# pierrebarbera/epa-ng

Hardware: AMD Instinct MI355X
Metric: query placements/sec (whole node), 512-tip GTR+G4 DNA ref, preplace+thorough (higher is better)
Workload: dtype f64; 1 GPU; cfg2: 512-tip DNA GTR+G4 ref, W=1500, 150 bp reads, dyn-heur 0.99999, preplace+thorough; branches=1021, parallelism=query-shard x1 (weak)

## Files before the change

### epa_ng_amd/api.py

```python
import ctypes as C
import os

import numpy as np

HERE = os.path.dirname(os.path.abspath(__file__))
DEV_SO = os.environ.get("EPA_DEV_SO", os.path.join(HERE, "libepa_dev.so"))

__all__ = ["EpaError", "dev_lib", "device_count", "encode_queries", "Evaluator", "PAIR_DTYPE",
           "RESULT_DTYPE", "ROW_DTYPE", "DEV_SO", "Packed4", "pack_codes_4bit", "unpack_codes_4bit", "Comm",
           "comm_unique_id", "mapped_rccl_path", "comm_set_library", "comm_library_path", "comm_set_default_timeout",
           "pci_id_str", "FLAG_LOOKUP_BLOCKS", "FLAG_LOOKUP_AUTO", "LOOKUP_RESIDENT", "LOOKUP_BLOCKS", "ERR_NO_MEMORY",
           "footprint", "lookup_plan", "set_mem_cap", "quadrature_legendre01", "quadrature_laguerre", "posterior_rule",
           "profile_from_phred"]

FLAG_LOOKUP_BLOCKS = 0x40
FLAG_LOOKUP_AUTO = 0x80
LOOKUP_RESIDENT = 0
LOOKUP_BLOCKS = 1
ERR_NO_MEMORY = -10

PAIR_DTYPE = np.dtype([("branch_id", np.uint32), ("seq_id", np.uint32)])
RESULT_DTYPE = np.dtype([("lnl", np.float64), ("pendant_length", np.float64),
                         ("distal_length", np.float64)])

ROW_DTYPE = np.dtype([("branch_id", np.uint32), ("seq_id", np.uint32), ("lnl", np.float64),
                      ("pendant_length", np.float64), ("distal_length", np.float64)])


class EpaError(RuntimeError):
    def __init__(self, code, msg):
        super().__init__("epa_dev error %d: %s" % (code, msg))
        self.code = code


class _RefDesc(C.Structure):
    _fields_ = [("states", C.c_uint32), ("rate_cats", C.c_uint32), ("sites", C.c_uint32),
                ("branches", C.c_uint32),
                ("eigenvals", C.c_void_p), ("eigenvecs_u", C.c_void_p),
                ("eigenvecs_uinv", C.c_void_p), ("freqs", C.c_void_p), ("rates", C.c_void_p),
                ("rate_weights", C.c_void_p), ("prop_invar", C.c_double),
                ("prox_clv", C.c_void_p), ("prox_scaler", C.c_void_p), ("dist_clv", C.c_void_p),
                ("dist_tipchars", C.c_void_p), ("dist_scaler", C.c_void_p),
                ("branch_length", C.c_void_p),
                ("tipmap", C.c_void_p), ("tipmap_size", C.c_uint32),
                ("blo_min_branch", C.c_double), ("blo_max_branch", C.c_double),
                ("blo_default_branch", C.c_double), ("blo_epsilon", C.c_double),
                ("pendant_default", C.c_double), ("blo_max_rounds", C.c_uint32),
                ("blo_max_newton", C.c_uint32), ("flags", C.c_uint32), ("aa_x_as_n", C.c_uint32),
                ("invariant_state", C.c_void_p)]


class _Stats(C.Structure):
    _fields_ = [("pairs", C.c_uint64), ("rounds", C.c_uint64), ("newton_evals", C.c_uint64),
                ("reverts", C.c_uint64)]


class _Footprint(C.Structure):
    _fields_ = [(n, C.c_uint64) for n in ("reft", "scsum", "lookup", "lookup2", "refi", "misc", "create_temp",
                                          "reference", "bank", "steady", "peak")]


_LIB = None


def dev_lib():
    global _LIB
    if _LIB is None:
        if not os.path.exists(DEV_SO):
            raise ImportError("libepa_dev.so is missing: run `python __graft_entry__.py` "
                              "(build()) -- the HIP extension is the only compute path")
        try:
            import torch
            if torch.cuda.is_available():
                torch.cuda.init()
        except ImportError:
            pass
        L = C.CDLL(DEV_SO)
        L.epa_dev_device_count.restype = C.c_int
        L.epa_dev_create.argtypes = [C.POINTER(_RefDesc), C.c_int, C.POINTER(C.c_void_p)]
        L.epa_dev_destroy.argtypes = [C.c_void_p]
        L.epa_dev_last_error.restype = C.c_char_p
        L.epa_dev_last_error.argtypes = [C.c_void_p]
        L.epa_dev_set_stream.argtypes = [C.c_void_p, C.c_void_p]
        L.epa_dev_build_lookup.argtypes = [C.c_void_p]
        L.epa_dev_set_option.argtypes = [C.c_void_p, C.c_char_p, C.c_int]
        L.epa_encode_queries.argtypes = [C.c_uint32, C.c_uint32, C.c_uint32,
                                         C.POINTER(C.c_char_p), C.c_int, C.c_int, C.c_void_p,
                                         C.c_void_p, C.c_void_p, C.POINTER(C.c_uint32)]
        L.epa_encode_queries_compact.argtypes = [C.c_uint32, C.c_uint32, C.c_uint32,
                                                 C.POINTER(C.c_char_p), C.c_int, C.c_int, C.c_uint32,
                                                 C.c_void_p, C.c_void_p, C.c_void_p,
                                                 C.POINTER(C.c_uint32)]
        L.epa_dev_set_query_layout.argtypes = [C.c_void_p, C.c_uint32]
        L.epa_dev_preplace.argtypes = [C.c_void_p, C.c_void_p, C.c_void_p, C.c_void_p, C.c_uint32,
                                       C.c_void_p]
        L.epa_dev_preplace_bounded.argtypes = [C.c_void_p, C.c_void_p, C.c_void_p, C.c_void_p, C.c_uint32, C.c_uint32,
                                               C.c_void_p, C.c_void_p]
        L.epa_dev_thorough.argtypes = [C.c_void_p, C.c_void_p, C.c_uint64, C.c_void_p, C.c_void_p,
                                       C.c_void_p, C.c_uint32, C.c_void_p, C.POINTER(_Stats)]
        L.epa_dev_score_at.argtypes = [C.c_void_p, C.c_void_p, C.c_void_p, C.c_void_p, C.c_void_p, C.c_uint64,
                                       C.c_void_p, C.c_void_p, C.c_void_p, C.c_uint32, C.c_void_p]
        L.epa_dev_site_lnl.argtypes = [C.c_void_p, C.c_void_p, C.c_void_p, C.c_void_p, C.c_void_p, C.c_uint64,
                                       C.c_void_p, C.c_void_p, C.c_void_p, C.c_uint32, C.c_uint32, C.c_void_p]
        L.epa_dev_rell_support.argtypes = [C.c_void_p, C.c_void_p, C.c_void_p, C.c_void_p, C.c_void_p, C.c_uint64,
                                           C.c_void_p, C.c_void_p, C.c_void_p, C.c_uint32, C.c_void_p, C.c_uint32,
                                           C.c_uint64, C.c_void_p]
        L.epa_dev_rell_tests.argtypes = L.epa_dev_rell_support.argtypes + [C.c_void_p, C.c_void_p]
        L.epa_dev_rell_au.argtypes = L.epa_dev_rell_support.argtypes[:-1] + [C.c_void_p, C.c_uint32, C.c_void_p, C.c_void_p,
                                                                             C.c_void_p]
        L.epa_dev_rell_kh.argtypes = L.epa_dev_rell_tests.argtypes
        L.epa_dev_marginal_like.argtypes = [C.c_void_p, C.c_void_p, C.c_uint64, C.c_void_p, C.c_void_p, C.c_uint32,
                                            C.c_void_p, C.c_void_p, C.c_uint32, C.c_void_p, C.c_void_p, C.c_void_p,
                                            C.c_uint32, C.c_void_p, C.c_void_p]
        L.epa_dev_preplace_profile.argtypes = [C.c_void_p, C.c_void_p, C.c_uint32, C.c_void_p, C.c_void_p, C.c_uint32,
                                               C.c_void_p]
        L.epa_dev_thorough_profile.argtypes = [C.c_void_p, C.c_void_p, C.c_uint64, C.c_void_p, C.c_uint32, C.c_void_p,
                                               C.c_void_p, C.c_uint32, C.c_void_p, C.POINTER(_Stats)]
        L.epa_dev_score_at_profile.argtypes = [C.c_void_p, C.c_void_p, C.c_void_p, C.c_void_p, C.c_void_p, C.c_uint64,
                                               C.c_void_p, C.c_uint32, C.c_void_p, C.c_void_p, C.c_uint32, C.c_void_p]
        L.epa_dev_site_lnl_profile.argtypes = [C.c_void_p, C.c_void_p, C.c_void_p, C.c_void_p, C.c_void_p, C.c_uint64,
                                               C.c_void_p, C.c_uint32, C.c_void_p, C.c_void_p, C.c_uint32, C.c_uint32,
                                               C.c_void_p]
        L.epa_dev_place_chunk_profile.argtypes = [C.c_void_p, C.c_void_p, C.c_uint32, C.c_void_p, C.c_void_p, C.c_uint32,
                                                  C.c_double, C.c_void_p, C.c_void_p, C.c_uint64, C.POINTER(C.c_uint64),
                                                  C.POINTER(_Stats)]
        L.epa_profile_from_phred.argtypes = [C.c_uint32, C.c_uint32, C.c_uint32, C.c_void_p, C.c_void_p, C.c_void_p,
                                             C.c_void_p]
        L.epa_quadrature_legendre01.argtypes = [C.c_uint32, C.c_void_p, C.c_void_p]
        L.epa_quadrature_laguerre.argtypes = [C.c_uint32, C.c_void_p, C.c_void_p]
        L.epa_dev_set_heuristic.argtypes = [C.c_void_p, C.c_int, C.c_double]
        L.epa_dev_set_query_packing.argtypes = [C.c_void_p, C.c_int]
        L.epa_pack_codes_4bit.argtypes = [C.c_void_p, C.c_uint32, C.c_uint32, C.c_void_p]
        L.epa_unpack_codes_4bit.argtypes = [C.c_void_p, C.c_uint32, C.c_uint32, C.c_void_p]
        L.epa_dev_select_candidates.argtypes = [C.c_void_p, C.c_void_p, C.c_uint32, C.c_double,
                                                C.c_void_p, C.c_uint64, C.POINTER(C.c_uint64)]
        L.epa_dev_place_chunk.argtypes = [C.c_void_p, C.c_void_p, C.c_void_p, C.c_void_p, C.c_uint32,
                                          C.c_uint32, C.c_double, C.c_void_p, C.c_void_p,
                                          C.c_uint64, C.POINTER(C.c_uint64), C.POINTER(_Stats)]
        L.epa_dev_dedup_queries.argtypes = [C.c_void_p, C.c_void_p, C.c_void_p, C.c_void_p, C.c_uint32, C.c_void_p,
                                            C.c_void_p, C.POINTER(C.c_uint32)]
        L.epa_dev_place_chunk_dedup.argtypes = [C.c_void_p, C.c_void_p, C.c_void_p, C.c_void_p, C.c_uint32, C.c_uint32,
                                                C.c_double, C.c_void_p, C.c_void_p, C.c_uint64, C.POINTER(C.c_uint64),
                                                C.POINTER(_Stats), C.c_void_p, C.c_void_p, C.POINTER(C.c_uint32)]
        L.epa_dev_chunk_stage.argtypes = [C.c_void_p, C.c_int, C.c_void_p, C.c_void_p, C.c_void_p, C.c_uint32]
        L.epa_dev_chunk_launch.argtypes = [C.c_void_p, C.c_int, C.c_uint32, C.c_double, C.c_void_p,
                                           C.c_void_p, C.c_uint64, C.c_uint32]
        L.epa_dev_chunk_launch_begin.argtypes = [C.c_void_p, C.c_int, C.c_uint32, C.c_double, C.c_void_p,
                                           C.c_void_p, C.c_uint64, C.c_uint32]
        L.epa_dev_chunk_launch_end.argtypes = [C.c_void_p, C.c_int]
        L.epa_dev_chunk_launch_many_begin.argtypes = [C.c_void_p, C.POINTER(C.c_int), C.c_int, C.c_uint32, C.c_double,
                                                      C.c_uint64, C.c_uint32]
        L.epa_dev_chunk_launch_many.argtypes = L.epa_dev_chunk_launch_many_begin.argtypes
        L.epa_dev_chunk_finish.argtypes = [C.c_void_p, C.c_int, C.POINTER(C.c_void_p),
                                           C.POINTER(C.c_void_p), C.POINTER(C.c_uint64), C.POINTER(_Stats)]
        L.epa_dev_tree_logl.argtypes = [C.c_void_p, C.c_uint32, C.POINTER(C.c_double)]
        L.epa_dev_place_all.argtypes = [C.c_void_p, C.c_void_p, C.c_void_p, C.c_void_p, C.c_uint32,
                                        C.c_uint32, C.c_double, C.c_int, C.c_uint32, C.c_uint32,
                                        C.c_void_p, C.c_void_p, C.c_void_p, C.c_void_p,
                                        C.POINTER(_Stats)]
        L.epa_comm_get_unique_id.argtypes = [C.c_void_p]
        L.epa_comm_create.argtypes = [C.c_void_p, C.c_void_p, C.c_int, C.c_int, C.c_uint32, C.c_int,
                                      C.POINTER(C.c_void_p)]
        L.epa_comm_destroy.argtypes = [C.c_void_p]
        L.epa_comm_destroy.restype = None
        L.epa_dev_gather_results.argtypes = [C.c_void_p, C.c_void_p, C.c_void_p, C.c_void_p, C.c_uint64,
                                             C.c_uint32, C.POINTER(C.c_uint64)]
        L.epa_dev_gather_slot.argtypes = [C.c_void_p, C.c_void_p, C.c_int, C.c_uint32, C.POINTER(C.c_uint64)]
        L.epa_comm_collect.argtypes = [C.c_void_p, C.c_uint64, C.POINTER(C.c_void_p), C.POINTER(C.c_uint32),
                                       C.POINTER(C.c_uint64)]
        L.epa_comm_flush.argtypes = [C.c_void_p, C.c_void_p, C.POINTER(C.c_uint64), C.POINTER(C.c_uint32)]
        L.epa_comm_carried_rows.argtypes = [C.c_void_p]
        L.epa_comm_carried_rows.restype = C.c_uint64
        L.epa_dev_gather_rows.argtypes = [C.c_void_p, C.c_void_p, C.c_void_p, C.c_uint64, C.POINTER(C.c_uint64)]
        L.epa_dev_place_all_rows.argtypes = [C.c_void_p, C.c_void_p, C.c_void_p, C.c_void_p, C.c_uint32, C.c_uint32, C.c_double,
                                             C.c_int, C.c_uint32, C.c_uint32, C.c_uint32, C.POINTER(C.c_void_p),
                                             C.POINTER(C.c_uint64), C.c_void_p]
        L.epa_comm_abort.argtypes = [C.c_void_p]
        L.epa_comm_abort.restype = None
        L.epa_comm_set_library.argtypes = [C.c_char_p]
        L.epa_comm_library_path.restype = C.c_char_p
# ... 189 lines not shown
                    held.append(a)
                    arr[i] = a.ctypes.data
            return arr, held

        pc, h1 = ptr_array(prox_clv, np.float64)
        dc, h2 = ptr_array(dist_clv, np.float64)
        ps, h3 = ptr_array(prox_scaler, np.uint32)
        ds, h4 = ptr_array(dist_scaler, np.uint32)
        dt, h5 = ptr_array(dist_tip, np.uint8)
        tm = np.ascontiguousarray(tipmap, dtype=np.uint32) if tipmap is not None else None
        d = _RefDesc()
        d.states, d.rate_cats, d.sites, d.branches = states, self.c, W, B
        d.eigenvals, d.eigenvecs_u, d.eigenvecs_uinv = (keep[0].ctypes.data, keep[1].ctypes.data,
                                                       keep[2].ctypes.data)
        d.freqs, d.rates, d.rate_weights = keep[3].ctypes.data, keep[4].ctypes.data, keep[5].ctypes.data
        d.prop_invar = float(pinv)
        inv = None
        if invariant_state is not None:
            inv = np.ascontiguousarray(invariant_state, dtype=np.int8)
            d.invariant_state = inv.ctypes.data
        d.prox_clv = C.cast(pc, C.c_void_p)
        d.prox_scaler = C.cast(ps, C.c_void_p)
        d.dist_clv = C.cast(dc, C.c_void_p)
        d.dist_tipchars = C.cast(dt, C.c_void_p) if dist_tip is not None else None
        d.dist_scaler = C.cast(ds, C.c_void_p)
        d.branch_length = keep[6].ctypes.data
        if tm is not None:
            d.tipmap, d.tipmap_size = tm.ctypes.data, len(tm)
        d.aa_x_as_n = int(aa_x_as_n)
        d.flags = int(flags)
        h = C.c_void_p()
        rc = L.epa_dev_create(C.byref(d), device, C.byref(h))
        if rc:
            raise EpaError(rc, L.epa_dev_last_error(None).decode())
        self.h = h
        self.L = L
        self.last_stats = None

    def close(self):
        if getattr(self, "h", None):
            self.L.epa_dev_destroy(self.h)
            self.h = None

    def __del__(self):
        self.close()

    def _check(self, rc):
        if rc:
            raise EpaError(rc, self.L.epa_dev_last_error(self.h).decode())

    def set_stream(self, stream_ptr):
        self._check(self.L.epa_dev_set_stream(self.h, stream_ptr))

    def set_option(self, key, value=1):
        self._check(self.L.epa_dev_set_option(self.h, key.encode(), int(value)))

    def build_lookup(self):
        self._check(self.L.epa_dev_build_lookup(self.h))

    def _layout(self, codes):
        packed = isinstance(codes, Packed4)
        row = codes.stride if packed else (int(codes.shape[1]) if len(codes.shape) == 2 else self.W)
        self._check(self.L.epa_dev_set_query_layout(self.h, 0 if row == self.W else row))
        self._check(self.L.epa_dev_set_query_packing(self.h, 4 if packed else 8))

    def preplace(self, codes, win_begin, win_span, Q=None, out=None):
        Q = len(win_begin) if Q is None else Q
        if out is None:
            out = np.empty((Q, self.B), np.float64)
        self._layout(codes)
        self._check(self.L.epa_dev_preplace(self.h, _ptr(codes), _ptr(win_begin), _ptr(win_span),
                                            Q, _ptr(out)))
        return out

    def preplace_bounded(self, codes, win_begin, win_span, max_span, seg_keys=False):
        Q = len(win_begin)
        out = np.empty((Q, self.B), np.float64)
        keys = np.zeros((Q, ((self.B + 63) // 64 + 7) // 8 * 8), np.uint64) if seg_keys else None
        self._layout(codes)
        self._check(self.L.epa_dev_preplace_bounded(self.h, _ptr(codes), _ptr(win_begin), _ptr(win_span), Q,
                                                    int(max_span), _ptr(out), _ptr(keys)))
        return (out, keys) if seg_keys else out

    def thorough(self, pairs, codes, win_begin, win_span, Q=None, n_pairs=None, out=None):
        Q = len(win_begin) if Q is None else Q
        n = len(pairs) if n_pairs is None else n_pairs
        if out is None:
            out = np.empty(n, RESULT_DTYPE)
        st = _Stats()
        self._layout(codes)
        self._check(self.L.epa_dev_thorough(self.h, _ptr(pairs), n, _ptr(codes), _ptr(win_begin),
                                            _ptr(win_span), Q, _ptr(out), C.byref(st)))
        self.last_stats = {"pairs": st.pairs, "rounds": st.rounds,
                           "newton_evals": st.newton_evals, "reverts": st.reverts}
        return out

    def _entries(self, pairs, pendant, distal, proximal, codes, win_begin, Q, stream_id=None):
        n, Q = len(pairs), (len(win_begin) if Q is None else Q)
        host = (np.ndarray, list, tuple)
        pendant, distal, proximal = (np.ascontiguousarray(a, dtype=np.float64) if isinstance(a, host) else a
                                     for a in (pendant, distal, proximal))
        if isinstance(stream_id, host):
            stream_id = np.ascontiguousarray(stream_id, dtype=np.uint64)
        self._layout(codes)
        return n, Q, pendant, distal, proximal, stream_id

    @staticmethod
    def _want(who, want, table):
        want = tuple(want)
        unknown = [w for w in want if w not in table]
        if unknown:
            raise ValueError("%s: unknown output %r" % (who, unknown[0]))
        return {w: np.empty(*table[w]) for w in want}

    def score_at(self, pairs, pendant, distal, codes, win_begin, win_span, proximal=None, Q=None, out=None):
        n, Q, pendant, distal, proximal, _ = self._entries(pairs, pendant, distal, proximal, codes, win_begin, Q)
        if out is None:
            out = np.empty(n, np.float64)
        self._check(self.L.epa_dev_score_at(self.h, _ptr(pairs), _ptr(pendant), _ptr(distal), _ptr(proximal), n,
                                            _ptr(codes), _ptr(win_begin), _ptr(win_span), Q, _ptr(out)))
        return out

    def site_lnl(self, pairs, pendant, distal, codes, win_begin, win_span, proximal=None, pitch=None, Q=None, out=None):
        n, Q, pendant, distal, proximal, _ = self._entries(pairs, pendant, distal, proximal, codes, win_begin, Q)
        if pitch is None:
            pitch = int(np.max(np.asarray(win_span)[:Q])) if Q else 0
        if out is None:
            out = np.empty((n, int(pitch)), np.float64)
        self._check(self.L.epa_dev_site_lnl(self.h, _ptr(pairs), _ptr(pendant), _ptr(distal), _ptr(proximal), n,
                                            _ptr(codes), _ptr(win_begin), _ptr(win_span), Q, int(pitch), _ptr(out)))
        return out

    def marginal_like(self, pairs, codes, win_begin, win_span, x_frac, x_logw, p_len, p_logw, Q=None, out=None, grid=False):
        n, Q = self._entries(pairs, None, None, None, codes, win_begin, Q)[:2]
        x_frac, x_logw, p_len, p_logw = (np.ascontiguousarray(a, dtype=np.float64) for a in (x_frac, x_logw, p_len, p_logw))
        if x_frac.shape != x_logw.shape or p_len.shape != p_logw.shape or x_frac.ndim != 1 or p_len.ndim != 1:
            raise ValueError("marginal_like: nodes and log weights must be 1-d arrays of equal length")
        Kx, Kp = len(x_frac), len(p_len)
        if out is None:
            out = np.empty(n, np.float64)
        g = np.empty((n, Kx, Kp), np.float64) if grid else None
        self._check(self.L.epa_dev_marginal_like(self.h, _ptr(pairs), n, _ptr(x_frac), _ptr(x_logw), Kx, _ptr(p_len),
                                                 _ptr(p_logw), Kp, _ptr(codes), _ptr(win_begin), _ptr(win_span), Q,
                                                 _ptr(out), _ptr(g)))
        return (out, g) if grid else out

    def rell_support(self, pairs, pendant, distal, codes, win_begin, win_span, replicates, seed=1, stream_id=None,
                     proximal=None, Q=None, out=None):
        n, Q, pendant, distal, proximal, stream_id = self._entries(pairs, pendant, distal, proximal, codes, win_begin, Q,
                                                                   stream_id)
        if out is None:
            out = np.empty(n, np.float64)
        self._check(self.L.epa_dev_rell_support(self.h, _ptr(pairs), _ptr(pendant), _ptr(distal), _ptr(proximal), n,
                                                _ptr(codes), _ptr(win_begin), _ptr(win_span), Q, _ptr(stream_id),
                                                int(replicates), int(seed), _ptr(out)))
        return out

    def rell_tests(self, pairs, pendant, distal, codes, win_begin, win_span, replicates, seed=1, stream_id=None,
                   proximal=None, want=("support", "elw", "p_sh"), Q=None):
        out = self._want("rell_tests", want, {w: ((len(pairs),), np.float64) for w in ("support", "elw", "p_sh")})
        n, Q, pendant, distal, proximal, stream_id = self._entries(pairs, pendant, distal, proximal, codes, win_begin, Q,
                                                                   stream_id)
        self._check(self.L.epa_dev_rell_tests(self.h, _ptr(pairs), _ptr(pendant), _ptr(distal), _ptr(proximal), n,
                                              _ptr(codes), _ptr(win_begin), _ptr(win_span), Q, _ptr(stream_id),
                                              int(replicates), int(seed), _ptr(out.get("support")), _ptr(out.get("elw")),
                                              _ptr(out.get("p_sh"))))
# ... 405 lines not shown
```

### epa_ng_amd/csrc/chunk.hip

```cpp
#include "epa_dev_internal.hpp"

#include <string.h>

#include <algorithm>

static int chunk_body_begin(epa_ctx* ctx, const uint8_t* d_codes, const uint32_t* d_begin, const uint32_t* d_span,
                            uint32_t Q, uint32_t max_span, double threshold, epa_pair* d_pairs,
                            uint64_t max_pairs, uint32_t* rb, SelectPending* sp, epa_result* d_res = nullptr,
                            unsigned long long* d_stats = nullptr) {
  const uint32_t pitch = (ctx->B + 7u) & ~7u;
  PreTable t{(double*)epa_scratch(ctx, SLOT_TABLE, sizeof(double) * (size_t)Q * pitch), pitch};
  if (!t.lnl) return epa_fail(ctx, EPA_ERR_HIP, "hipMalloc(chunk table)");
  const uint32_t nseg = (ctx->B + 63) / 64;
  if (nseg <= 64 && ctx->heur_mode == 0) {
    t.segp = (nseg + 7u) & ~7u;
    t.segmax = (unsigned long long*)epa_scratch(ctx, SLOT_SEGMAX, sizeof(unsigned long long) * (size_t)Q * t.segp);
    if (!t.segmax) return epa_fail(ctx, EPA_ERR_HIP, "hipMalloc(segment maxima)");
  }
  const uint32_t* pre_status = nullptr;
  int rc = launch_preplace(ctx, d_codes, d_begin, d_span, Q, t, max_span, &pre_status);
  if (!rc) rc = launch_select_begin(ctx, t, pre_status, Q, threshold, d_pairs, max_pairs, d_span, rb, sp);
  const bool behind_rb = !rc && d_stats && sp->d_rb && sp->bitmap && max_pairs <= 0xffffffffull;
  if (behind_rb) {
    rc = launch_select_emit(ctx, sp);
    if (!rc) rc = epa_zero_async(ctx, d_stats, 128, epa_th_ctr(ctx), epa_th_ctr(ctx) ? 64 : 0);
    if (!rc) {
      ctx->clean_stats[ctx->bank] = d_stats;
      ctx->clean_ctr[ctx->bank] = epa_th_ctr(ctx) != nullptr;
    }
  }
  if (behind_rb && !rc && d_res) {
    const bool off = !ctx->opt.queued_thorough;
    const int cls = epa_span_class(ctx->s, max_span);
    const bool eligible = !off && ctx->s == 4 && !ctx->generic_thorough && ctx->dna.ng == 1 && epa_th_ctr(ctx) &&
                          epa_tip_class_ok(cls);
    if (eligible) {
      rc = launch_select_emit(ctx, sp);
      if (!rc && ctx->clean_stats[ctx->bank] == d_stats) ctx->clean_stats[ctx->bank] = nullptr;
      else if (!rc) rc = epa_zero_async(ctx, d_stats, 128);
      if (!rc) {
        const int q = launch_thorough_queued(ctx, d_pairs, sp->d_rb, max_pairs, d_codes, d_begin, d_span, max_span, d_res, d_stats);
        if (q == -2) return EPA_ERR_HIP;
        sp->queued_cls = q;
      }
    }
  }
  return rc;
}

static int chunk_body_end(epa_ctx* ctx, SelectPending* sp, const uint8_t* d_codes, const uint32_t* d_begin,
                          const uint32_t* d_span, uint32_t max_span, epa_pair* d_pairs, epa_result* d_res,
                          unsigned long long* d_stats, uint64_t* n_out) {
  uint64_t n = 0;
  int rc = launch_select_end(ctx, sp, &n);
  if (rc) return rc;
  rc = select_check_status(ctx, sp);
  if (rc) return rc;
  *n_out = n;
  if (sp->queued_cls >= 0 && sp->rb[RB_HIST + sp->queued_cls] + sp->rb[RB_HIST + epa_tip_class(sp->queued_cls)] == (uint32_t)n) return EPA_OK;
  if (ctx->clean_stats[ctx->bank] == d_stats && sp->queued_cls < 0) ctx->clean_stats[ctx->bank] = nullptr;
  else {
    ctx->clean_stats[ctx->bank] = nullptr;
    rc = epa_zero_async(ctx, d_stats, 128);
    if (rc) return rc;
  }
  if (n == 0) return EPA_OK;
  const bool hist_ok = sp->have_hist && (sp->tip_split || !epa_tipd_active(ctx));
  return launch_thorough(ctx, d_pairs, n, d_codes, d_begin, d_span, max_span, d_res, d_stats,
                         hist_ok ? sp->cls_hist : nullptr);
}

static int chunk_body(epa_ctx* ctx, const uint8_t* d_codes, const uint32_t* d_begin, const uint32_t* d_span,
                      uint32_t Q, uint32_t max_span, double threshold, epa_pair* d_pairs, epa_result* d_res,
                      uint64_t max_pairs, unsigned long long* d_stats, uint64_t* n_out) {
  uint32_t rb[64] = {};
  SelectPending sp;
  int rc = chunk_body_begin(ctx, d_codes, d_begin, d_span, Q, max_span, threshold, d_pairs, max_pairs, rb, &sp, d_res, d_stats);
  if (rc) return rc;
  return chunk_body_end(ctx, &sp, d_codes, d_begin, d_span, max_span, d_pairs, d_res, d_stats, n_out);
}

int chunk_stats(epa_ctx* ctx, uint64_t n, const unsigned long long* hst, epa_thorough_stats* stats) {
  epa_xcd_feedback(ctx, n, hst);
  ctx->last_stats.pairs = n;
  ctx->last_stats.rounds = hst[0];
  ctx->last_stats.newton_evals = hst[1];
  ctx->last_stats.reverts = hst[2];
  if (stats) *stats = ctx->last_stats;
  if (hst[3])
    return epa_fail(ctx, EPA_ERR_NEG_INF,
                    "-INF logl at branch " + std::to_string((uint32_t)(hst[4] >> 32)) +
                        " with sequence " + std::to_string((uint32_t)(hst[4] & 0xffffffffu)));
  return EPA_OK;
}

extern "C" int epa_dev_place_chunk(epa_ctx* ctx, const uint8_t* q_codes, const uint32_t* win_begin,
                                   const uint32_t* win_span, uint32_t Q, uint32_t max_span,
                                   double threshold, epa_pair* pairs, epa_result* results,
                                   uint64_t max_pairs, uint64_t* n_pairs, epa_thorough_stats* stats) {
  if (!ctx || !q_codes || !win_begin || !win_span || !pairs || !results || !n_pairs)
    return epa_fail(ctx, EPA_ERR_INVALID_ARG, "null argument");
// ... 460 lines not shown
```

### epa_ng_amd/csrc/epa_dev.hip

```cpp
#include "epa_dev_internal.hpp"

#include <math.h>
#include <string.h>

#include <algorithm>
#include <numeric>
#include <atomic>
#include <thread>

static thread_local std::string g_create_err;

int epa_fail(epa_ctx* ctx, int code, const std::string& msg) {
  if (ctx) ctx->err = msg; else g_create_err = msg;
  return code;
}

namespace {
__global__ void __launch_bounds__(256) k_zero(uint4* __restrict__ a, size_t na, uint4* __restrict__ b, size_t nb) {
  const size_t stride = (size_t)gridDim.x * 256, i0 = (size_t)blockIdx.x * 256 + threadIdx.x;
  const uint4 z = make_uint4(0u, 0u, 0u, 0u);
  for (size_t i = i0; i < na; i += stride) a[i] = z;
  for (size_t i = i0; i < nb; i += stride) b[i] = z;
}
}
// ... 481 lines not shown
}

extern "C" int epa_quadrature_legendre01(uint32_t K, double* nodes, double* log_weights) {
  if (K < 1 || K > 64 || !nodes || !log_weights) return EPA_ERR_INVALID_ARG;
  std::vector<double> d(K, 0.0), o(K > 1 ? K - 1 : 0), x;
  for (uint32_t i = 1; i < K; ++i) o[i - 1] = (double)i / std::sqrt(4.0 * i * i - 1.0);
  tridiag_eigenvalues(d, o, x);
  for (uint32_t j = 0; j < K; ++j) {
    double t = x[j], dp = 1.0;
    for (int it = 0; it < 3; ++it) {
      double p0 = 1.0, p1 = t;
      for (uint32_t n = 1; n < K; ++n) { const double p2 = ((2.0 * n + 1.0) * t * p1 - n * p0) / (n + 1.0); p0 = p1; p1 = p2; }
      dp = K * (t * p1 - p0) / (t * t - 1.0);
      if (it < 2) t -= p1 / dp;
    }
    nodes[j] = 0.5 * (1.0 + t);
    log_weights[j] = -std::log((1.0 - t) * (1.0 + t)) - 2.0 * std::log(std::fabs(dp));
  }
  const double norm = log_sum_exp(log_weights, K);
  for (uint32_t j = 0; j < K; ++j) log_weights[j] -= norm;
  return EPA_OK;
}

extern "C" int epa_quadrature_laguerre(uint32_t K, double* nodes, double* log_weights) {
  if (K < 1 || K > 64 || !nodes || !log_weights) return EPA_ERR_INVALID_ARG;
  std::vector<double> d(K), o(K > 1 ? K - 1 : 0), x;
  for (uint32_t i = 0; i < K; ++i) d[i] = 2.0 * i + 1.0;
  for (uint32_t i = 1; i < K; ++i) o[i - 1] = (double)i;
  tridiag_eigenvalues(d, o, x);
  for (uint32_t j = 0; j < K; ++j) {
    double t = x[j], lm = 1.0;
    for (int it = 0; it < 3; ++it) {
      double l0 = 1.0, l1 = 1.0 - t;
      for (uint32_t n = 1; n < K; ++n) { const double l2 = ((2.0 * n + 1.0 - t) * l1 - n * l0) / (n + 1.0); l0 = l1; l1 = l2; }
      lm = l0;
      if (it < 2) t -= l1 * t / (K * (l1 - l0));
    }
    nodes[j] = t;
    log_weights[j] = std::log(t) - 2.0 * std::log((double)K) - 2.0 * std::log(std::fabs(lm));
  }
  const double norm = log_sum_exp(log_weights, K);
  for (uint32_t j = 0; j < K; ++j) log_weights[j] -= norm;
  return EPA_OK;
}

extern "C" int epa_dev_device_count(void) {
  int n = 0;
  if (hipGetDeviceCount(&n) != hipSuccess) { (void)hipGetLastError(); return 0; }
  return n;
}

extern "C" const char* epa_dev_last_error(const epa_ctx* ctx) {
  return ctx ? ctx->err.c_str() : g_create_err.c_str();
}

extern "C" int epa_dev_set_query_layout(epa_ctx* ctx, uint32_t code_stride) {
  if (!ctx) return EPA_ERR_INVALID_ARG;
  ctx->code_stride = code_stride;
  return EPA_OK;
}

extern "C" int epa_dev_set_option(epa_ctx* ctx, const char* key, int value) {
  if (!ctx || !key) return EPA_ERR_INVALID_ARG;
  if (strcmp(key, "lookup_block") == 0) {
    if (!ctx->lookup_blocks) return epa_fail(ctx, EPA_ERR_INVALID_ARG, "set_option: lookup_block needs a context in the blocked lookup layout");
    if (value <= 0 || (value & 63)) return epa_fail(ctx, EPA_ERR_INVALID_ARG, "set_option: lookup_block must be a positive multiple of 64");
    for (void* p : ctx->blk_buf)
      if (p) return epa_fail(ctx, EPA_ERR_INVALID_ARG, "set_option: lookup_block must be set before the first preplacement");
    ctx->lookup_block = (uint32_t)value;
    return EPA_OK;
  }
  const bool dedup_key = strcmp(key, "dedup_key_bits") == 0;
  if (dedup_key || strcmp(key, "dedup_sort_bits") == 0) {
    if (value < 0 || value > 64) return epa_fail(ctx, EPA_ERR_INVALID_ARG, std::string("set_option: ") + key + " must be 0 .. 64");
    (dedup_key ? ctx->opt.dedup_key_bits : ctx->opt.dedup_sort_bits) = value;
    return EPA_OK;
  }
  struct Entry { const char* name; int EpaOptions::*field; };
  static const Entry table[] = {
      {"thorough_generic", &EpaOptions::thorough_generic}, {"preplace_generic", &EpaOptions::preplace_generic},
      {"select_full_rows", &EpaOptions::select_full_rows}, {"select_sort", &EpaOptions::select_sort},
      {"queued_thorough", &EpaOptions::queued_thorough},   {"xcd_balance", &EpaOptions::xcd_balance},
      {"aa_valu", &EpaOptions::aa_valu},                   {"timers", &EpaOptions::timers},
      {"newton_lds", &EpaOptions::newton_lds},             {"tip_distal", &EpaOptions::tip_distal}};
  for (const Entry& e : table)
    if (strcmp(key, e.name) == 0) {
      ctx->opt.*e.field = value;
      ctx->generic_thorough = ctx->generic_native || ctx->opt.thorough_generic != 0;
      return EPA_OK;
    }
  return epa_fail(ctx, EPA_ERR_INVALID_ARG, std::string("set_option: unknown key '") + key + "'");
}

extern "C" int epa_dev_set_heuristic(epa_ctx* ctx, int mode, double param) {
  if (!ctx) return EPA_ERR_INVALID_ARG;
  if (mode < EPA_HEUR_DYNAMIC || mode > EPA_HEUR_BASEBALL)
    return epa_fail(ctx, EPA_ERR_INVALID_ARG, "set_heuristic: unknown mode");
  if (mode == EPA_HEUR_FIXED && !(param >= 0.0 && param <= 1.0))
    return epa_fail(ctx, EPA_ERR_INVALID_ARG, "set_heuristic: the fraction must lie in [0, 1]");
  ctx->heur_mode = mode;
  ctx->heur_param = param;
  return EPA_OK;
}

extern "C" int epa_dev_set_query_packing(epa_ctx* ctx, int bits) {
  if (!ctx) return EPA_ERR_INVALID_ARG;
  if (bits != 8 && bits != 4) return epa_fail(ctx, EPA_ERR_INVALID_ARG, "set_query_packing: 8 or 4 bits per code");
  if (bits == 4 && ctx->s != 4)
    return epa_fail(ctx, EPA_ERR_UNSUPPORTED, "set_query_packing: the 4-bit format holds nucleotide codes only");
  ctx->code_packed4 = bits == 4;
  return EPA_OK;
}

extern "C" int epa_pack_codes_4bit(const uint8_t* codes, uint32_t Q, uint32_t stride, uint8_t* packed) {
  if (!codes || !packed) return EPA_ERR_INVALID_ARG;
  const size_t ps = ((size_t)stride + 1) / 2;
  const unsigned cap = g_encode_threads.load(std::memory_order_relaxed);
  const unsigned hw = cap ? cap : std::max(1u, std::thread::hardware_concurrency());
  const unsigned nt = (unsigned)std::min<uint64_t>(std::min(hw, 32u), std::max<uint64_t>(1, (uint64_t)Q * stride >> 20));
  std::vector<int> bad(nt, 0);
  auto work = [&](unsigned t) {
    const uint32_t q0 = (uint32_t)((uint64_t)Q * t / nt), q1 = (uint32_t)((uint64_t)Q * (t + 1) / nt);
    unsigned over = 0;
    for (uint32_t q = q0; q < q1; ++q) {
      const uint8_t* r = codes + (size_t)q * stride;
      uint8_t* o = packed + (size_t)q * ps;
      for (uint32_t p = 0; p < stride / 2; ++p) {
        const uint8_t hi = r[2 * p], lo = r[2 * p + 1];
        over |= hi | lo;
        o[p] = (uint8_t)((hi << 4) | lo);
      }
      if (stride & 1) { const uint8_t hi = r[stride - 1]; over |= hi; o[ps - 1] = (uint8_t)(hi << 4); }
    }
    bad[t] = over > 15;
  };
  if (nt == 1) work(0);
  else {
    std::vector<std::thread> th;
    for (unsigned t = 0; t < nt; ++t) th.emplace_back(work, t);
    for (auto& x : th) x.join();
  }
  for (unsigned t = 0; t < nt; ++t) if (bad[t]) return EPA_ERR_INVALID_ARG;
  return EPA_OK;
}

extern "C" int epa_unpack_codes_4bit(const uint8_t* packed, uint32_t Q, uint32_t stride, uint8_t* codes) {
  if (!codes || !packed) return EPA_ERR_INVALID_ARG;
  const size_t ps = ((size_t)stride + 1) / 2;
  for (uint32_t q = 0; q < Q; ++q)
    for (uint32_t i = 0; i < stride; ++i) {
      const uint8_t b = packed[(size_t)q * ps + i / 2];
      codes[(size_t)q * stride + i] = (i & 1) ? (b & 15u) : (b >> 4);
    }
  return EPA_OK;
}

extern "C" int epa_dev_set_stream(epa_ctx* ctx, void* s) {
  if (!ctx) return EPA_ERR_INVALID_ARG;
  ctx->stream = (hipStream_t)s;
  return EPA_OK;
}

extern "C" void epa_dev_destroy(epa_ctx* ctx) {
  if (!ctx) return;
  (void)hipSetDevice(ctx->device);
  (void)hipDeviceSynchronize();
  for (int i = 0; i < epa_ctx::N_BANKS * epa_ctx::N_SCRATCH; ++i) if (ctx->scratch[i]) (void)hipFree(ctx->scratch[i]);
  if (ctx->refT) (void)hipFree(ctx->refT);
  if (ctx->scSum) (void)hipFree(ctx->scSum);
  if (ctx->blen) (void)hipFree(ctx->blen);
  if (ctx->lookup) (void)hipFree(ctx->lookup);
  if (ctx->lookup2) (void)hipFree(ctx->lookup2);
  if (ctx->prof_tab) (void)hipFree(ctx->prof_tab);
  for (void* p : ctx->blk_buf) if (p) (void)hipFree(p);
  for (auto& v : ctx->blk_ev) for (hipEvent_t e : v) if (e) (void)hipEventDestroy(e);
  if (ctx->th_ctr) (void)hipFree(ctx->th_ctr);
  for (hipEvent_t e : ctx->ev_rb) if (e) (void)hipEventDestroy(e);
  if (ctx->refI) (void)hipFree(ctx->refI);
  if (ctx->cinv) (void)hipFree(ctx->cinv);
  if (ctx->resc0) (void)hipFree(ctx->resc0);
  if (ctx->tip_row) (void)hipFree(ctx->tip_row);
  if (ctx->tipmask) (void)hipFree(ctx->tipmask);
  if (ctx->tipd) (void)hipFree(ctx->tipd);
  for (hipStream_t st : ctx->side_stream) if (st) (void)hipStreamDestroy(st);
  for (hipEvent_t e : ctx->ev_fork) if (e) (void)hipEventDestroy(e);
  for (hipEvent_t e : ctx->ev_join) if (e) (void)hipEventDestroy(e);
  if (ctx->dmodel) (void)hipFree(ctx->dmodel);
  for (ChunkSlot& sl : ctx->slots) {
    if (sl.h_in) (void)hipHostFree(sl.h_in);
    if (sl.h_out) (void)hipHostFree(sl.h_out);
    if (sl.h_stats) (void)hipHostFree(sl.h_stats);
    if (sl.h_sel) (void)hipHostFree(sl.h_sel);
    if (sl.d_in) (void)hipFree(sl.d_in);
    if (sl.d_unpacked) (void)hipFree(sl.d_unpacked);
    if (sl.d_pairs) (void)hipFree(sl.d_pairs);
    if (sl.d_res) (void)hipFree(sl.d_res);
    if (sl.d_stats) (void)hipFree(sl.d_stats);
    if (sl.d_merge) (void)hipFree(sl.d_merge);
    if (sl.d_gpairs) (void)hipFree(sl.d_gpairs);
    if (sl.d_gres) (void)hipFree(sl.d_gres);
    if (sl.d_goff) (void)hipFree(sl.d_goff);
    if (sl.h_goff) (void)hipHostFree(sl.h_goff);
    for (hipEvent_t e : {sl.ev_up, sl.ev_done, sl.ev_down, sl.ev_base}) if (e) (void)hipEventDestroy(e);
    if (sl.stream) (void)hipStreamDestroy(sl.stream);
  }
  if (ctx->copy_stream) (void)hipStreamDestroy(ctx->copy_stream);
  if (ctx->down_stream) (void)hipStreamDestroy(ctx->down_stream);
  std::vector<EvTimer*> ts = {&ctx->t_lookup};
  for (auto& bk : ctx->t_bank) for (auto& t : bk) ts.push_back(&t);
  for (auto* t : ts) { if (t->a) (void)hipEventDestroy(t->a); if (t->b) (void)hipEventDestroy(t->b); }
  delete ctx;
}

static int precompute_from_tree(epa_ctx* ctx, const epa_tree_desc* t, const uint32_t* d_tipmap);

static int padded_cats(int s, int c_in, uint32_t flags, bool from_tree) {
  int c = (c_in == 1 || c_in == 2) ? 4 : c_in;
  if (s == 4 && c_in >= 3 && (c_in & 3)) c = (c_in + 3) & ~3;
  if (s == 20 && (c_in == 3 || (c_in >= 5 && c_in <= 7))) c = (c_in + 3) & ~3;
  if (c_in >= 3 && c != c_in && (flags & EPA_FLAG_RATE_SCALERS) && !from_tree) c = c_in;
  return c;
}

static bool tuned_thorough_shape(int s, int c, uint32_t flags, bool zero0) {
  const bool sliding = !(flags & EPA_FLAG_RAXML_BLO);
  const bool dna_groups = s == 4 && (c & 3) == 0 && c <= 16;
  const bool tuned_local = (s == 4 && zero0) || s == 20;
  const bool tuned_cats = c == 4 || (dna_groups && sliding && zero0) || (s == 20 && c == 8);
  return tuned_cats && (sliding || tuned_local) &&
         !(flags & (EPA_FLAG_NEWTON_SLOW_BISECT | EPA_FLAG_NEWTON_STRICT_DF | EPA_FLAG_KEEP_EIGENVALUES));
}

static std::atomic<uint64_t> g_mem_cap{0};
extern "C" void epa_dev_set_mem_cap(uint64_t bytes) { g_mem_cap.store(bytes, std::memory_order_relaxed); }

constexpr uint32_t EPA_BLOCK_DEFAULT = 1024;
constexpr int EPA_PLAN_BANKS = 4;

extern "C" int epa_dev_footprint(uint32_t states, uint32_t rate_cats, uint64_t sites, uint64_t branches, int flags,
                                 int from_tree, uint32_t block_branches, int banks, epa_footprint* out) {
  if (!out || !(states == 4 || states == 20) || rate_cats < 1 || rate_cats > EPA_MAX_CATS || !sites || !branches ||
      sites > 0xffffffffull || branches > 0xffffffffull || banks < 0 || (block_branches & 63u))
    return epa_fail(nullptr, EPA_ERR_INVALID_ARG, "footprint: bad shape");
  const uint64_t s = states, W = sites, B = branches;
  const uint64_t c = (uint64_t)padded_cats((int)states, (int)rate_cats, (uint32_t)flags, from_tree != 0);
  const bool blocks = (flags & EPA_FLAG_LOOKUP_BLOCKS) != 0;
  const bool tuned = tuned_thorough_shape((int)s, (int)c, (uint32_t)flags, !(flags & EPA_FLAG_KEEP_EIGENVALUES));
  epa_footprint f;
  memset(&f, 0, sizeof(f));
  f.reft = 8 * 2 * B * c * s * W;
  f.scsum = 4 * B * W;
  if (!blocks) {
    f.lookup = 8 * B * W * (s == 4 ? 16 : 24);
    f.lookup2 = s == 4 ? 8 * B * 2 * ((W + 1) / 2) * 36 : 0;
    f.refi = tuned ? 8 * B * c * s * W + B * W : 0;
// ... 679 lines not shown
}

extern "C" int epa_dev_build_lookup(epa_ctx* ctx) {
  if (!ctx) return EPA_ERR_INVALID_ARG;
  if (ctx->lookup_built || ctx->lookup_blocks) return EPA_OK;
  EPA_HIP(ctx, hipSetDevice(ctx->device));
  int rc = launch_build_lookup(ctx);
  if (rc) return rc;
  EPA_HIP(ctx, hipStreamSynchronize(ctx->stream));
  ctx->lookup_built = true;
  return EPA_OK;
}

const uint32_t* host_view(const uint32_t* p, size_t n, std::vector<uint32_t>& buf, hipStream_t st) {
  if (!epa_is_device_ptr(p)) return p;
  buf.resize(n);
  (void)hipStreamSynchronize(st);
  if (hipMemcpy(buf.data(), p, n * sizeof(uint32_t), hipMemcpyDeviceToHost) != hipSuccess)
    return nullptr;
  return buf.data();
}

static int check_windows(epa_ctx* ctx, const uint32_t* hb, const uint32_t* hs, uint32_t Q,
                         uint32_t* max_span, bool allow_empty = false) {
  uint32_t mx = 0;
  for (uint32_t q = 0; q < Q; ++q) {
    if (hs[q] == 0 && !allow_empty)
      return epa_fail(ctx, EPA_ERR_QUERY_ALL_GAP,
                      "Sequence " + std::to_string(q) + " does not appear to have any non-gap sites!");
    if ((uint64_t)hb[q] + hs[q] > ctx->W)
      return epa_fail(ctx, EPA_ERR_QUERY_WIDTH,
                      "Query sequence length not same as reference alignment!");
    mx = std::max(mx, hs[q]);
  }
  if (ctx->code_stride && mx > ctx->code_stride)
    return epa_fail(ctx, EPA_ERR_INVALID_ARG, "a window is longer than the compact code stride");
  *max_span = mx;
  return EPA_OK;
}

extern "C" int epa_dev_preplace(epa_ctx* ctx, const uint8_t* q_codes, const uint32_t* win_begin,
                                const uint32_t* win_span, uint32_t Q, double* lnl) {
  return epa_dev_preplace_bounded(ctx, q_codes, win_begin, win_span, Q, 0, lnl, nullptr);
}

extern "C" int epa_dev_preplace_bounded(epa_ctx* ctx, const uint8_t* q_codes, const uint32_t* win_begin,
                                        const uint32_t* win_span, uint32_t Q, uint32_t max_span, double* lnl,
                                        uint64_t* seg_keys) {
  if (!ctx || !q_codes || !win_begin || !win_span || !lnl)
    return epa_fail(ctx, EPA_ERR_INVALID_ARG, "null argument");
  if (Q == 0) return EPA_OK;
  EPA_HIP(ctx, hipSetDevice(ctx->device));
  int rc = epa_dev_build_lookup(ctx);
  if (rc) return rc;
  if (max_span > ctx->W) max_span = ctx->W;
  if (max_span && !epa_is_device_ptr(win_span))
    for (uint32_t q = 0; q < Q; ++q)
      if (win_span[q] > max_span) return epa_fail(ctx, EPA_ERR_INVALID_ARG, "preplace: a window is longer than max_span");
  const uint32_t nseg = (ctx->B + 63) / 64, segp = (nseg + 7u) & ~7u;
  unsigned long long* d_seg = nullptr;
  if (seg_keys) {
    if (nseg > 64) return epa_fail(ctx, EPA_ERR_INVALID_ARG, "preplace: segment maxima exist up to 4096 branches");
    d_seg = (unsigned long long*)epa_scratch(ctx, SLOT_SEGMAX, sizeof(unsigned long long) * (size_t)Q * segp);
    if (!d_seg) return epa_fail(ctx, EPA_ERR_HIP, "hipMalloc(segment maxima)");
  }
  const uint8_t* d_codes = epa_codes_to_device(ctx, q_codes, Q);
  const uint32_t* d_begin = (const uint32_t*)epa_to_device(ctx, SLOT_BEGIN, win_begin, sizeof(uint32_t) * Q);
  const uint32_t* d_span = (const uint32_t*)epa_to_device(ctx, SLOT_SPAN, win_span, sizeof(uint32_t) * Q);
  if (!d_codes || !d_begin || !d_span) return epa_fail(ctx, EPA_ERR_HIP, "query upload failed");
  const bool out_dev = epa_is_device_ptr(lnl);
  double* d_lnl = out_dev ? lnl : (double*)epa_scratch(ctx, SLOT_TABLE, sizeof(double) * (size_t)Q * ctx->B);
  if (!d_lnl) return epa_fail(ctx, EPA_ERR_HIP, "hipMalloc(lnl)");
  const uint32_t* d_status = nullptr;
  rc = launch_preplace(ctx, d_codes, d_begin, d_span, Q, PreTable{d_lnl, ctx->B, d_seg, segp}, max_span, &d_status);
  if (rc) return rc;
  if (!out_dev)
    EPA_HIP(ctx, hipMemcpyAsync(lnl, d_lnl, sizeof(double) * (size_t)Q * ctx->B,
                                hipMemcpyDeviceToHost, ctx->stream));
  if (d_seg)
    EPA_HIP(ctx, hipMemcpyAsync(seg_keys, d_seg, sizeof(unsigned long long) * (size_t)Q * segp,
                                epa_is_device_ptr(seg_keys) ? hipMemcpyDeviceToDevice : hipMemcpyDeviceToHost, ctx->stream));
  EPA_HIP(ctx, hipStreamSynchronize(ctx->stream));
  return preplace_check_status(ctx, d_status);
}

extern "C" int epa_dev_thorough(epa_ctx* ctx, const epa_pair* pairs, uint64_t n_pairs,
                                const uint8_t* q_codes, const uint32_t* win_begin,
                                const uint32_t* win_span, uint32_t Q, epa_result* out,
                                epa_thorough_stats* stats) {
  if (!ctx || !q_codes || !win_begin || !win_span || (n_pairs && (!pairs || !out)))
    return epa_fail(ctx, EPA_ERR_INVALID_ARG, "null argument");
  if (stats) memset(stats, 0, sizeof(*stats));
  if (n_pairs == 0) return EPA_OK;
  EPA_HIP(ctx, hipSetDevice(ctx->device));
  if (ctx->refI) {
    int brc = epa_dev_build_lookup(ctx);
    if (brc) return brc;
  }
  std::vector<uint32_t> hb_buf, hs_buf;
  const uint32_t* hb = host_view(win_begin, Q, hb_buf, ctx->stream);
  const uint32_t* hs = host_view(win_span, Q, hs_buf, ctx->stream);
  if (!hb || !hs) return epa_fail(ctx, EPA_ERR_HIP, "cannot read window arrays");
  uint32_t max_span = 0;
  int rc = check_windows(ctx, hb, hs, Q, &max_span);
  if (rc) return rc;
  if (!epa_is_device_ptr(pairs)) {
    for (uint64_t i = 0; i < n_pairs; ++i)
      if (pairs[i].branch_id >= ctx->B || pairs[i].seq_id >= Q)
        return epa_fail(ctx, EPA_ERR_INVALID_ARG, "pair index out of range");
  }
  const uint8_t* d_codes = epa_codes_to_device(ctx, q_codes, Q);
  const uint32_t* d_begin = (const uint32_t*)epa_to_device(ctx, SLOT_BEGIN, win_begin, sizeof(uint32_t) * Q);
  const uint32_t* d_span = (const uint32_t*)epa_to_device(ctx, SLOT_SPAN, win_span, sizeof(uint32_t) * Q);
  const epa_pair* d_pairs = (const epa_pair*)epa_to_device(ctx, SLOT_PAIRS, pairs, sizeof(epa_pair) * n_pairs);
  if (!d_codes || !d_begin || !d_span || !d_pairs)
    return epa_fail(ctx, EPA_ERR_HIP, "thorough input upload failed");
  const bool out_dev = epa_is_device_ptr(out);
  epa_result* d_out = out_dev ? out : (epa_result*)epa_scratch(ctx, SLOT_RESULTS, sizeof(epa_result) * n_pairs);
  unsigned long long* d_stats = (unsigned long long*)epa_scratch(ctx, SLOT_STATS, 256);
  if (!d_out || !d_stats) return epa_fail(ctx, EPA_ERR_HIP, "hipMalloc(thorough out)");
  rc = epa_zero_async(ctx, d_stats, 128);
  if (rc) return rc;
  rc = launch_thorough(ctx, d_pairs, n_pairs, d_codes, d_begin, d_span, max_span, d_out, d_stats);
  if (rc) return rc;
  unsigned long long hst[16];
  if (!out_dev)
    EPA_HIP(ctx, hipMemcpyAsync(out, d_out, sizeof(epa_result) * n_pairs, hipMemcpyDeviceToHost,
                                ctx->stream));
  if (!out_dev || stats) {
    EPA_HIP(ctx, hipMemcpyAsync(hst, d_stats, 128, hipMemcpyDeviceToHost, ctx->stream));
    EPA_HIP(ctx, hipStreamSynchronize(ctx->stream));
    return chunk_stats(ctx, n_pairs, hst, stats);
  }
  return EPA_OK;
}


namespace {

struct EntryArgs {
  const epa_pair* pairs;
  const double *pendant, *distal, *proximal;
  uint64_t n;
  const uint8_t* q_codes;
  const uint32_t *win_begin, *win_span;
  uint32_t Q;
  const double* prof = nullptr;
  uint32_t prof_stride = 0;
};

struct EntryCall {
  epa_ctx* ctx;
  const char* who;
  EntryArgs a;
  EntryStage st;
  std::vector<uint32_t> hb_buf, hs_buf;
  const uint64_t* d_sid = nullptr;
  bool empty = false;
  struct Out { void *user, *dev; size_t bytes; } out[3] = {};
  int n_out = 0;

  int stage() {
    const uint32_t* hb = host_view(a.win_begin, a.Q, hb_buf, ctx->stream);
    st.h_span = host_view(a.win_span, a.Q, hs_buf, ctx->stream);
    if (!hb || !st.h_span) return epa_fail(ctx, EPA_ERR_HIP, "cannot read window arrays");
    int rc = a.prof ? (int)EPA_OK : check_windows(ctx, hb, st.h_span, a.Q, &st.max_span, true);
// ... 558 lines not shown
```

### epa_ng_amd/csrc/epa_dev_internal.hpp

```cpp
#pragma once

#include <hip/hip_runtime.h>
#include <stdint.h>

#include <string>
#include <vector>

#include <rocprim/device/device_radix_sort.hpp>

#include "epa_dev.h"

using epa_radix_cfg = rocprim::radix_sort_config<rocprim::default_config, rocprim::default_config,
                                                 rocprim::default_config, 0>;

#define EPA_MAX_STATES 20
#define EPA_MAX_CATS 16
#define EPA_MAX_COLS 24
#define EPA_GRID_Y 65535u

struct ModelDNA {
  double U[16];
  double Ui[16];
  double lam[4];
  double rate[16];
  double w[16];
  double pi[4];
  int ng;
};

struct BloConsts {
  double min_branch, max_branch, default_branch, epsilon, pendant_default;
  uint32_t max_rounds, max_newton;
  uint32_t sliding;
  uint32_t newton_variant;
};

struct ModelDev {
  int s, c, ncols;
  double U[EPA_MAX_STATES * EPA_MAX_STATES];
  double Ui[EPA_MAX_STATES * EPA_MAX_STATES];
  double lam[EPA_MAX_STATES];
  double pi[EPA_MAX_STATES];
  double rate[EPA_MAX_CATS];
  double w[EPA_MAX_CATS];
  uint32_t colmask[EPA_MAX_COLS];
  double qt[EPA_MAX_COLS * EPA_MAX_STATES];
};

struct EvTimer {
  hipEvent_t a = nullptr, b = nullptr;
  bool valid = false;
};

constexpr int EPA_N_CLS = 12;
constexpr int EPA_N_CLSX = 17;

enum EpaReadback : int {
  RB_TOTAL = 0,
  RB_STATUS = RB_TOTAL + 1,
  RB_HIST = RB_STATUS + 8,
  RB_TIP_SPLIT = 30,
  RB_WINDOW = 32,
  RB_WORDS = RB_WINDOW + 4,
};
enum EpaSelStatus : int {
  SEL_OVERFLOW = 2,
  SEL_HIST = 8,
  SEL_TIP_TOTAL = 40,
  SEL_READBACK = 64,
  SEL_WORDS = 128,
};
static_assert(RB_TOTAL == 0 && RB_STATUS == 1 && RB_HIST == 9 && RB_TIP_SPLIT == 30 && RB_WINDOW == 32 && RB_WORDS == 36,
              "the read-back block's layout is shared with queued kernels: move a word everywhere or nowhere");
static_assert(RB_HIST + EPA_N_CLSX <= RB_TIP_SPLIT && RB_TIP_SPLIT < RB_WINDOW, "read-back fields overlap");
static_assert(SEL_HIST == 8 && SEL_TIP_TOTAL == 40 && SEL_READBACK == 64, "the selection's status block moved");
static_assert(RB_HIST - RB_STATUS == SEL_HIST, "k_pack_readback copies status words and histogram in one run");
static_assert(SEL_HIST + EPA_N_CLS <= SEL_TIP_TOTAL && SEL_TIP_TOTAL < SEL_READBACK && SEL_READBACK + RB_WORDS <= SEL_WORDS,
              "status block fields overlap");

struct PreTable {
  double* lnl = nullptr;
  uint32_t pitch = 0;
  unsigned long long* segmax = nullptr;
  uint32_t segp = 0;
};

struct SelectPending {
  PreTable table;
  const uint32_t* pre_status = nullptr;
  uint32_t Q = 0, cap = 0;
  double threshold = 0.0;
  epa_pair* d_pairs = nullptr;
  uint64_t max_pairs = 0;
  const uint32_t* d_span = nullptr;
  unsigned long long *stage = nullptr, *keys_a = nullptr, *keys_b = nullptr;
  uint32_t *counts = nullptr, *offsets = nullptr;
  uint32_t *bitmap = nullptr, *boffs = nullptr;
  uint32_t wpr = 0;
  void* temp = nullptr;
  size_t sort_bytes = 0;
  uint32_t* rb = nullptr;
  bool have_status = false;
  hipEvent_t ev_rb = nullptr;
  const uint32_t* d_rb = nullptr;
  bool emitted = false;
  int queued_cls = -1;
  uint32_t cls_hist[EPA_N_CLSX] = {};
  bool have_hist = false;
  bool tip_split = false;
};

enum class SlotState : int {
  Free,
  Staged,
  Begun,
  Launched,
  GroupMember,
};
constexpr int EPA_MAX_GROUP = 8;

struct ChunkInputs {
  const uint8_t* codes;
  const uint32_t *begin, *span;
};

struct __attribute__((visibility("hidden"))) ChunkSlot {
  void* h_in = nullptr;
  size_t h_in_sz = 0;
  void* d_in = nullptr;
  const uint8_t* x_codes = nullptr;
  const uint32_t* x_begin = nullptr;
  const uint32_t* x_span = nullptr;
  size_t d_in_sz = 0;
  uint8_t* d_unpacked = nullptr;
  size_t d_unpacked_sz = 0;
  size_t codes_bytes = 0;
  uint32_t Q = 0, stride = 0;
  bool packed4 = false;
  epa_pair* d_pairs = nullptr;
  epa_result* d_res = nullptr;
  size_t d_pairs_sz = 0, d_res_sz = 0;
  void* h_out = nullptr;
  size_t h_out_sz = 0;
  unsigned long long* h_stats = nullptr;
  unsigned long long* d_stats = nullptr;
  hipEvent_t ev_up = nullptr, ev_done = nullptr, ev_down = nullptr, ev_base = nullptr;
  hipStream_t stream = nullptr;
  const epa_pair* out_pairs = nullptr;
  const epa_result* out_res = nullptr;
  uint64_t n = 0;
  SlotState state = SlotState::Free;
  bool unfinished() const { return state == SlotState::Begun || state == SlotState::Launched || state == SlotState::GroupMember; }
  ChunkInputs staged_inputs() const {
    if (x_codes) return {x_codes, x_begin, x_span};
    const char* d = (const char*)d_in;
    const uint32_t* b = (const uint32_t*)(d + codes_bytes);
    return {(const uint8_t*)d, b, b + Q};
  }
  SelectPending sel;
  uint32_t* h_sel = nullptr;
  const uint8_t* l_codes = nullptr;
  const uint32_t *l_begin = nullptr, *l_span = nullptr;
  epa_pair* l_pairs = nullptr;
  epa_result* l_res = nullptr;
  uint32_t l_max_span = 0, l_flags = 0;
  int leader = -1;
  int g_index = 0;
  int g_n = 0;
  int g_left = 0;
  int g_slots[EPA_MAX_GROUP] = {};
  uint32_t g_qoff[EPA_MAX_GROUP + 1] = {};
  uint32_t own_Q = 0;
  const uint8_t* own_x_codes = nullptr;
  const uint32_t *own_x_begin = nullptr, *own_x_span = nullptr;
  void* d_merge = nullptr;
  size_t d_merge_sz = 0;
  epa_pair* d_gpairs = nullptr;
  epa_result* d_gres = nullptr;
  size_t g_cap = 0;
  uint32_t* d_goff = nullptr;
  uint32_t* h_goff = nullptr;

  void lead_merged(uint32_t total, const uint8_t* codes, const uint32_t* begin, const uint32_t* span) {
    own_Q = Q; own_x_codes = x_codes; own_x_begin = x_begin; own_x_span = x_span;
    Q = total; x_codes = codes; x_begin = begin; x_span = span;
  }
  void restore_own() { Q = own_Q; x_codes = own_x_codes; x_begin = own_x_begin; x_span = own_x_span; }
  void group_begun(ChunkSlot* all, const int* slots, int n, const uint32_t* qoff) {
    g_n = n;
    for (int i = 0; i <= n; ++i) g_qoff[i] = qoff[i];
    for (int i = 0; i < n; ++i) {
      g_slots[i] = slots[i];
      all[slots[i]].leader = slots[0];
      all[slots[i]].g_index = i;
      if (i) all[slots[i]].state = SlotState::GroupMember;
    }
  }
  void group_launched(ChunkSlot* all) {
    restore_own();
    g_left = g_n;
    for (int i = 1; i < g_n; ++i) {
      all[g_slots[i]].state = SlotState::Launched;
      all[g_slots[i]].l_flags = l_flags;
    }
  }
  void launch_over(ChunkSlot* all, SlotState to) {
    state = to;
    if (g_n <= 1) return;
    restore_own();
    for (int i = 0; i < g_n; ++i) {
      all[g_slots[i]].leader = -1;
      if (i) all[g_slots[i]].state = to;
    }
    g_n = 0;
    g_left = 0;
  }
};

struct EpaOptions {
  int thorough_generic = 0;
  int preplace_generic = 0;
  int select_full_rows = 0;
  int select_sort = 0;
  int queued_thorough = 0;
  int xcd_balance = 1;
  int aa_valu = 0;
  int timers = 1;
  int newton_lds = 0;
  int tip_distal = 1;
  int dedup_key_bits = 64;
  int dedup_sort_bits = 32;
};

struct epa_ctx {
  int device = 0;
  EpaOptions opt;
  int n_cu = 256;
  hipStream_t stream = nullptr;
  std::string err;

  int s = 0, c = 0, ncols = 0;
  int c_in = 0;
  uint32_t W = 0, B = 0;
  ModelDev hmodel;
  ModelDev* dmodel = nullptr;
  ModelDNA dna;
  bool dna_zero0 = false;
  bool rate_scalers = false;
  bool generic_thorough = false;
  bool generic_native = false;
  BloConsts blo;
  int aa_x_as_n = 0;
  uint32_t code_stride = 0;

  double* refT = nullptr;
  uint32_t* scSum = nullptr;
  double* blen = nullptr;
  double* lookup = nullptr;
  double* refI = nullptr;
  uint8_t* resc0 = nullptr;
  double* cinv = nullptr;
  double inv_w0 = 0.0;
  double* lookup2 = nullptr;
  uint32_t* tip_row = nullptr;
  uint8_t* tipmask = nullptr;
  double* tipd = nullptr;
  bool lookup_built = false;
  double* prof_tab = nullptr;
  bool lookup_blocks = false;
  uint32_t lookup_block = 1024;
  std::vector<double> h_blen;

  static constexpr int N_SCRATCH = 26;
  static constexpr int N_SLOTS = 24;
  static constexpr int N_BANKS = 1 + N_SLOTS;
  int bank = 0;
  void* scratch[N_BANKS * N_SCRATCH] = {};
  size_t scratch_sz[N_BANKS * N_SCRATCH] = {};

  uint32_t select_cap = 64;
  uint32_t* th_ctr = nullptr;
  bool code_packed4 = false;
  int heur_mode = 0;
  double heur_param = 0.0;

  hipStream_t copy_stream = nullptr, down_stream = nullptr;
  ChunkSlot slots[N_SLOTS];

  enum { T_PREPLACE = 0, T_THOROUGH = 1, T_SELECT = 2, T_SCORE = 3, T_SITES = 4, T_RELL = 5, T_MARGINAL = 6, T_RELL_TESTS = 7, T_RELL_AU = 8, T_RELL_KH = 9, T_PREPLACE_PROFILE = 10, T_DEDUP = 11, N_TIMERS = 12 };
  EvTimer t_lookup;
  std::vector<hipEvent_t> blk_ev[N_BANKS];
  uint32_t blk_ev_n[N_BANKS] = {};
  void* blk_buf[N_BANKS] = {};
  size_t blk_sz[N_BANKS] = {};
  EvTimer t_bank[N_BANKS][N_TIMERS];
  uint32_t xcd_cum[9] = {0u, 1u << 17, 2u << 17, 3u << 17, 4u << 17, 5u << 17, 6u << 17, 7u << 17, 1u << 20};
  double xcd_w[8] = {0.125, 0.125, 0.125, 0.125, 0.125, 0.125, 0.125, 0.125};
  double last_sclk_mhz = 0.0;
  bool xstamp_ok = false;
  hipEvent_t ev_rb[N_BANKS] = {};
  hipStream_t side_stream[N_BANKS] = {};
  hipEvent_t ev_fork[N_BANKS] = {}, ev_join[N_BANKS] = {};
  const void* clean_stats[N_BANKS] = {};
  bool clean_ctr[N_BANKS] = {};
  int t_last[N_TIMERS] = {};
  epa_thorough_stats last_stats{};
};

int epa_fail(epa_ctx* ctx, int code, const std::string& msg);
void* epa_scratch(epa_ctx* ctx, int slot, size_t bytes);
inline size_t align256(size_t x) { return (x + 255) & ~(size_t)255; }
struct Carver {
  char* base = nullptr;
  size_t off = 0;
  void* tail(size_t bytes) { char* p = base ? base + off : nullptr; off += bytes; return p; }
  template <typename T> T* take(size_t n) { return static_cast<T*>(tail(align256(sizeof(T) * n))); }
};
inline uint32_t* epa_th_ctr(epa_ctx* ctx) { return ctx->th_ctr ? ctx->th_ctr + 64 * ctx->bank : nullptr; }
int epa_zero_async(epa_ctx* ctx, void* p, size_t bytes, void* p2 = nullptr, size_t bytes2 = 0);
inline int epa_th_ctr_reset(epa_ctx* ctx, size_t bytes = 64) {
  if (ctx->clean_ctr[ctx->bank]) { ctx->clean_ctr[ctx->bank] = false; return 0; }
  return epa_zero_async(ctx, epa_th_ctr(ctx), bytes);
}
bool epa_is_device_ptr(const void* p);
const void* epa_to_device(epa_ctx* ctx, int slot, const void* p, size_t bytes);
const uint8_t* epa_codes_to_device(epa_ctx* ctx, const uint8_t* q_codes, uint32_t Q);
__attribute__((visibility("hidden"))) void launch_unpack4(hipStream_t st, const uint8_t* d_packed, uint8_t* d_codes, uint32_t Q, uint32_t stride);
__attribute__((visibility("hidden"))) const uint32_t* host_view(const uint32_t* p, size_t n, std::vector<uint32_t>& buf, hipStream_t st);
void epa_xcd_feedback(epa_ctx* ctx, uint64_t n_pairs, const unsigned long long* hst);
__attribute__((visibility("hidden"))) int chunk_stats(epa_ctx* ctx, uint64_t n, const unsigned long long* hst, epa_thorough_stats* stats);
#define EPA_XSTAMP_MASK 0x7ffffffffffull
void epa_timer_start(epa_ctx* ctx, EvTimer& t);
void epa_timer_stop(epa_ctx* ctx, EvTimer& t);
inline EvTimer& epa_t(epa_ctx* ctx, int which) { ctx->t_last[which] = ctx->bank; return ctx->t_bank[ctx->bank][which]; }

#define EPA_HIP(ctx, call)                                                               \
  do {                                                                                    \
    hipError_t e__ = (call);                                                              \
    if (e__ != hipSuccess)                                                                \
      return epa_fail(ctx, EPA_ERR_HIP, std::string(#call) + ": " + hipGetErrorString(e__)); \
  } while (0)

enum EpaSlot : int {
  SLOT_CODES = 0,
  SLOT_BEGIN = 1,
  SLOT_SPAN = 2,
  SLOT_OUT = 3,
  SLOT_PAIRS = 4,
  SLOT_CLV_PROX = 0,
  SLOT_CLV_DIST = 1,
  SLOT_TIPMAP = 2,
  SLOT_SCALER_PROX = 3,
  SLOT_SCALER_DIST = 4,
  SLOT_TABLE = 3,
  SLOT_RESULTS = 5,
  SLOT_PREPLACE = 6,
  SLOT_STATS = 6,
  SLOT_SELECT = 7,
  SLOT_NEWTON = 7,
  SLOT_CLASS_SORT = 8,
  SLOT_TREE_LNL = 9,
  SLOT_TH_TIMING = 9,
  SLOT_SEGMAX = 10,
  SLOT_PACKED4 = 10,
  SLOT_ROWS_OUT = 11,
  SLOT_ROWS = 12,
  SLOT_PENDANT = 7,
  SLOT_DISTAL = 8,
  SLOT_PROXIMAL = 9,
  SLOT_MG_RULE = 7,
  SLOT_MG_WAVES = 9,
  SLOT_RELL_SORT = 13,
  SLOT_RELL_BOUNDS = 14,
  SLOT_RELL_GROUPS = 15,
  SLOT_RELL_ROWS = 16,
  SLOT_RELL_STREAMS = 17,
  SLOT_RELL_TESTS = 18,
  SLOT_RELL_AU = 19,
  SLOT_RELL_KH = 20,
  SLOT_PROFILE = 21,
  SLOT_PROFILE_EIGEN = 22,
  SLOT_DEDUP = 23,
  SLOT_DEDUP_IN = 24,
  SLOT_DEDUP_ROWS = 25,
};

struct EntryStage {
  const epa_pair* d_pairs = nullptr;
  const double *d_pen = nullptr, *d_dis = nullptr, *d_prx = nullptr;
  uint64_t n = 0;
  const uint8_t* d_codes = nullptr;
  const uint32_t *d_begin = nullptr, *d_span = nullptr;
  const uint32_t* h_span = nullptr;
  const double* d_qe = nullptr;
  uint32_t qe_stride = 0;
  uint32_t Q = 0;
  uint32_t max_span = 0;
};

__host__ __device__ inline bool epa_tip_class_ok(int cls) { return cls <= 2 || cls == 10 || cls == 11; }
__host__ __device__ inline int epa_tip_class(int cls) { return cls <= 2 ? 12 + cls : cls == 10 ? 15 : cls == 11 ? 16 : cls; }
__host__ __device__ inline int epa_base_class(int key) { return key < 12 ? key : key <= 14 ? key - 12 : key == 15 ? 10 : 11; }
inline bool epa_tipd_active(const epa_ctx* ctx) {
  return ctx->tip_row && ctx->opt.tip_distal && ctx->s == 4 && !ctx->generic_thorough && ctx->dna.ng == 1 &&
         ctx->dna_zero0 && ctx->blo.sliding && !ctx->cinv;
}
constexpr uint32_t EPA_AA_LDS_MAX_SPAN = 102;
__host__ __device__ inline int epa_span_class(int states, uint32_t span) {
  if (states != 4) return span <= 64 ? 0 : span <= 128 ? 1 : span <= 192 ? 2 : 3;
  if (span > 64 && span <= 96) return 10;
  if (span > 128 && span <= 160) return 11;
  const uint32_t nch = (span + 63) / 64;
  return nch <= 4 ? (nch ? (int)nch - 1 : 0) : nch <= 6 ? 4 : nch <= 8 ? 5 : nch <= 12 ? 6 : nch <= 16 ? 7 : nch <= 24 ? 8 : 9;
}

int launch_transform(epa_ctx* ctx, const double* d_clv_or_null, const uint8_t* d_tip_or_null,
                     const uint32_t* d_tipmap, uint32_t tipmap_size, double* dst);
int launch_build_lookup(epa_ctx* ctx);
int launch_build_lookup2(epa_ctx* ctx);
uint32_t epa_block_branches(const epa_ctx* ctx);
size_t epa_block_bytes(int s, uint32_t W, uint32_t blk, size_t* off2);
void* epa_block_buffer(epa_ctx* ctx);
int launch_build_lookup_block(epa_ctx* ctx, uint32_t b0, uint32_t nb, double* blk_lookup);
int launch_build_lookup2_block(epa_ctx* ctx, uint32_t nb, const double* blk_lookup, double* blk_lookup2);
int launch_preplace(epa_ctx* ctx, const uint8_t* d_codes, const uint32_t* d_begin, const uint32_t* d_span, uint32_t Q,
                    const PreTable& t, uint32_t max_span, const uint32_t** d_status);
int preplace_check_status(epa_ctx* ctx, const uint32_t* d_status);
__attribute__((visibility("hidden"))) int preplace_window_error(epa_ctx* ctx, const uint32_t* st);
__attribute__((visibility("hidden"))) void launch_scan_counts(epa_ctx* ctx, uint32_t* cnt, uint32_t K, const uint32_t* tip_row = nullptr,
                                                               uint32_t* tip_total = nullptr);
int launch_thorough(epa_ctx* ctx, const epa_pair* d_pairs, uint64_t n_pairs, const uint8_t* d_codes,
                    const uint32_t* d_begin, const uint32_t* d_span, uint32_t max_span,
                    epa_result* d_out, unsigned long long* d_stats,
                    const uint32_t* cls_hist = nullptr);
int launch_thorough_queued(epa_ctx* ctx, const epa_pair* d_pairs, const uint32_t* d_spec, uint64_t max_pairs,
                           const uint8_t* d_codes, const uint32_t* d_begin, const uint32_t* d_span, uint32_t max_span,
                           epa_result* d_out, unsigned long long* d_stats);
int launch_select_emit(epa_ctx* ctx, SelectPending* sp);
int launch_thorough_aa(epa_ctx* ctx, const epa_pair* d_pairs, const uint32_t* d_order, uint64_t n_pairs,
                       const uint8_t* d_codes, const uint32_t* d_begin, const uint32_t* d_span,
                       uint32_t max_span, bool want_lds, epa_result* d_out, unsigned long long* d_stats);
int launch_thorough_generic(epa_ctx* ctx, const epa_pair* d_pairs, uint64_t n_pairs, const uint8_t* d_codes,
                            const uint32_t* d_begin, const uint32_t* d_span, uint32_t max_span,
                            epa_result* d_out, unsigned long long* d_stats,
                            const uint32_t* d_order = nullptr, bool caller_times = false,
                            const double* d_qe = nullptr, uint32_t qe_stride = 0);
int launch_thorough_aa_mfma(epa_ctx* ctx, const epa_pair* d_pairs, const uint32_t* d_order, uint64_t n_pairs,
                            const uint8_t* d_codes, const uint32_t* d_begin, const uint32_t* d_span,
                            uint32_t max_span, epa_result* d_out, unsigned long long* d_stats);
__attribute__((visibility("hidden"))) uint32_t epa_column_mask(int s, int col);
__attribute__((visibility("hidden"))) int epa_profile_stage(epa_ctx* ctx, const char* who, const double* prof, uint32_t stride,
                                                            const uint32_t* hb, const uint32_t* hs, const uint32_t* d_span, uint32_t Q,
                                                            bool allow_empty, uint32_t* max_span, const double** d_prof, const double** d_qe);
int launch_score_at(epa_ctx* ctx, const EntryStage& e, double* d_lnl);
enum SiteLnlFlags : unsigned { SITES_PLAIN = 0u, SITES_PAD = 1u, SITES_TIMED = 2u };
int launch_site_lnl(epa_ctx* ctx, const EntryStage& e, const uint32_t* d_order, uint64_t n_rows, uint32_t pitch,
                    double* d_rows, unsigned flags);
struct RellDraws {
  const uint64_t* d_stream_id;
  uint32_t replicates;
  uint64_t seed;
};
int launch_rell(epa_ctx* ctx, const EntryStage& e, const RellDraws& dr, double* d_support);
int launch_rell_tests(epa_ctx* ctx, const EntryStage& e, const RellDraws& dr, double* d_support, double* d_elw, double* d_p_sh);
int launch_rell_au(epa_ctx* ctx, const EntryStage& e, const RellDraws& dr, const uint32_t* h_scale_pm, uint32_t n_scales,
                   double* d_p_au, uint32_t* d_counts, double* d_fit);
__attribute__((visibility("hidden"))) int launch_rell_kh(epa_ctx* ctx, const EntryStage& e, const RellDraws& dr, double* d_p_kh, double* d_p_wkh, double* d_p_wsh);
int launch_marginal(epa_ctx* ctx, const EntryStage& e, const double* d_rule, uint32_t Kx, uint32_t Kp, double* d_marginal,
                    double* d_grid);
int launch_select(epa_ctx* ctx, const PreTable& t, const uint32_t* pre_status, uint32_t Q, double threshold,
                  epa_pair* d_pairs, uint64_t max_pairs, uint64_t* n_pairs,
                  const uint32_t* d_span = nullptr);
int launch_select_begin(epa_ctx* ctx, const PreTable& t, const uint32_t* pre_status, uint32_t Q, double threshold,
                        epa_pair* d_pairs, uint64_t max_pairs, const uint32_t* d_span, uint32_t* rb, SelectPending* sp);
int launch_select_end(epa_ctx* ctx, SelectPending* sp, uint64_t* n_pairs);
int select_check_status(epa_ctx* ctx, const SelectPending* sp);
```

### epa_ng_amd/csrc/preplace.hip

```cpp
#include "epa_dev_internal.hpp"
#include "wave_util.hpp"

#include <cstdlib>
#include <cstring>

#include <algorithm>

namespace {

constexpr int GQ = 256;
constexpr int CH = 160;
constexpr int SPREAD = 96;
constexpr int TROWS = CH + SPREAD;
constexpr int NB = 16;
constexpr int CW = CH / 4;

struct Group {
  uint32_t start;
  uint32_t count;
  uint32_t min_begin;
  uint32_t cls;
};

__device__ __forceinline__ void validate_window(uint32_t i, uint32_t begin, uint32_t span, uint32_t W,
                                                uint32_t cmax, uint32_t* status) {
  if (span == 0) atomicMax(&status[0], 0x80000000u | i);
  else if ((uint64_t)begin + span > W || span > cmax) atomicMax(&status[1], 0x80000000u | i);
}
__global__ void k_validate(const uint32_t* __restrict__ win_begin, const uint32_t* __restrict__ win_span,
                           uint32_t Q, uint32_t W, uint32_t cmax, uint32_t* __restrict__ status) {
  const uint32_t i = blockIdx.x * blockDim.x + threadIdx.x;
  if (i < Q) validate_window(i, win_begin[i], win_span[i], W, cmax, status);
}

__global__ void k_iota(uint32_t* v, uint32_t n) {
  const uint32_t i = blockIdx.x * blockDim.x + threadIdx.x;
  if (i < n) v[i] = i;
}

__global__ void __launch_bounds__(256) k_count_keys(const uint32_t* __restrict__ keys, uint32_t Q,
                                                    uint32_t* __restrict__ cnt, uint32_t* __restrict__ rank) {
  const uint32_t q = blockIdx.x * 256 + threadIdx.x;
  if (q < Q) rank[q] = atomicAdd(&cnt[keys[q]], 1u);
}
__global__ void __launch_bounds__(1024) k_scan_counts(uint32_t* __restrict__ cnt, uint32_t K,
                                                      const uint32_t* __restrict__ tip_row = nullptr,
                                                      uint32_t* __restrict__ tip_total = nullptr) {
  __shared__ uint32_t wsum[16];
  __shared__ uint32_t carry_s;
  __shared__ uint32_t tips_s;
  const uint32_t t = threadIdx.x, lane = t & 63u, wv = t >> 6;
  if (t == 0) { carry_s = 0; tips_s = 0; }
  __syncthreads();
  constexpr uint32_t PER = 8;
  uint32_t tips = 0;
  for (uint32_t base = 0; base < K; base += 1024 * PER) {
    uint32_t v[PER], tot = 0;
#pragma unroll
    for (uint32_t i = 0; i < PER; ++i) {
      const uint32_t k = base + t * PER + i;
      v[i] = k < K ? cnt[k] : 0u;
      tot += v[i];
      if (tip_row && k + 1 < K && tip_row[k] != 0xffffffffu) tips += v[i];
    }
    uint32_t inc = tot;
#pragma unroll
    for (int o = 1; o < 64; o <<= 1) {
      const uint32_t u = __shfl_up(inc, o);
      if ((int)lane >= o) inc += u;
    }
    if (lane == 63) wsum[wv] = inc;
    __syncthreads();
    uint32_t before = carry_s;
    for (uint32_t w = 0; w < wv; ++w) before += wsum[w];
    uint32_t run = before + inc - tot;
#pragma unroll
    for (uint32_t i = 0; i < PER; ++i) {
      const uint32_t k = base + t * PER + i;
      if (k < K) cnt[k] = run;
      run += v[i];
    }
    __syncthreads();
    if (t == 1023) carry_s = run;
    __syncthreads();
  }
  if (tip_total) {
    if (tips) atomicAdd(&tips_s, tips);
    __syncthreads();
    if (t == 0) *tip_total = tips_s;
  }
}
__global__ void __launch_bounds__(256) k_scatter_sorted(const uint32_t* __restrict__ keys,
                                                        const uint32_t* __restrict__ rank,
                                                        const uint32_t* __restrict__ offs, uint32_t Q,
                                                        uint32_t* __restrict__ sorted_keys,
                                                        uint32_t* __restrict__ perm) {
  const uint32_t q = blockIdx.x * 256 + threadIdx.x;
  if (q >= Q) return;
  const uint32_t k = keys[q], pos = offs[k] + rank[q];
  sorted_keys[pos] = k;
  perm[pos] = q;
}

__global__ void __launch_bounds__(256) k_make_groups(const uint32_t* __restrict__ sorted_keys, uint32_t Q,
                                                     uint32_t Wp, uint32_t n_blocks,
                                                     uint32_t class_blocks, uint32_t gq0, uint32_t gq1,
                                                     uint32_t spr0, uint32_t max_runs, Group* __restrict__ groups,
                                                     uint32_t max_groups, uint32_t* __restrict__ status) {
  extern __shared__ uint32_t sh[];
  uint32_t* lo = sh;
  uint32_t* runbase = lo + n_blocks + 1;
  uint32_t* run_start = runbase + n_blocks + 1;
  uint32_t* run_end = run_start + max_runs;
  uint32_t* run_off = run_end + max_runs;
  auto lower_bound = [&](uint32_t a, uint32_t b, uint64_t key) {
    while (a < b) {
      const uint32_t m = (a + b) >> 1;
      if ((uint64_t)sorted_keys[m] < key) a = m + 1; else b = m;
    }
    return a;
  };
  for (uint32_t k = threadIdx.x; k <= n_blocks; k += blockDim.x)
    lo[k] = k == n_blocks ? Q : lower_bound(0, Q, (uint64_t)k * Wp);
  for (uint32_t i = threadIdx.x; i < max_groups; i += blockDim.x) groups[i] = Group{0, 0, 0, 0};
  __syncthreads();
  if (threadIdx.x == 0) {
    uint32_t r = 0;
    for (uint32_t b = 0; b < n_blocks; ++b) {
      const uint32_t gq = b >= class_blocks ? gq1 : gq0;
      runbase[b] = r;
      r += (lo[b + 1] - lo[b] + gq - 1) / gq;
    }
    runbase[n_blocks] = r;
  }
  __syncthreads();
  const uint32_t nruns = min(runbase[n_blocks], max_runs);
  for (uint32_t r = threadIdx.x; r < nruns; r += blockDim.x) {
    uint32_t b = 0;
    while (b + 1 < n_blocks && r >= runbase[b + 1]) ++b;
    const uint32_t gq = b >= class_blocks ? gq1 : gq0;
    const uint32_t start = lo[b] + (r - runbase[b]) * gq, end = min(lo[b + 1], start + gq);
    const uint32_t k0 = sorted_keys[start], k1 = sorted_keys[end - 1];
    const uint32_t spr = b >= class_blocks ? (uint32_t)SPREAD : spr0;
    run_start[r] = start;
    run_end[r] = end;
    run_off[r] = (k1 - k0 < spr) ? 1u : (k1 / spr - k0 / spr + 1);
  }
  __syncthreads();
  uint32_t* cnt = run_off + max_runs + 1;
  for (uint32_t r = threadIdx.x; r < nruns; r += blockDim.x) cnt[r] = run_off[r];
  __syncthreads();
  for (uint32_t r = threadIdx.x; r <= nruns; r += blockDim.x) {
    uint32_t g = 0;
    for (uint32_t i = 0; i < r; ++i) g += cnt[i];
    run_off[r] = g;
  }
  __syncthreads();
  if (threadIdx.x == 0) {
    const uint32_t r1 = class_blocks < n_blocks ? min(runbase[class_blocks], nruns) : nruns;
    status[4] = min(run_off[nruns], max_groups);
    status[5] = min(run_off[r1], max_groups);
  }
  for (uint32_t r = threadIdx.x; r < nruns; r += blockDim.x) {
    uint32_t b = 0;
    while (b + 1 < n_blocks && r >= runbase[b + 1]) ++b;
    const uint32_t cls = b >= class_blocks ? 1u : 0u;
    const uint32_t start = run_start[r], end = run_end[r], g0 = run_off[r], n = run_off[r + 1] - g0;
    if (n == 1) {
      if (g0 < max_groups) groups[g0] = Group{start, end - start, 0, cls};
    } else {
      const uint32_t spr = cls ? (uint32_t)SPREAD : spr0;
      const uint32_t kb = sorted_keys[start] / spr;
      uint32_t a = start;
      for (uint32_t k = 0; k < n; ++k) {
        const uint32_t e = k + 1 == n ? end : lower_bound(a, end, (uint64_t)(kb + k + 1) * spr);
        if (g0 + k < max_groups) groups[g0 + k] = Group{a, e - a, 0, cls};
        a = e;
      }
    }
  }
}

template <int NCOLS, bool ACC>
__global__ void __launch_bounds__(GQ, ACC ? 2 : 4) k_preplace(const double* __restrict__ lookup,
                                                 const uint8_t* __restrict__ codes,
                                                 const uint32_t* __restrict__ win_begin,
                                                 const uint32_t* __restrict__ win_span,
                                                 const uint32_t* __restrict__ perm,
                                                 const Group* __restrict__ groups, uint32_t W,
                                                 uint32_t cstride, uint32_t crel,
                                                 uint32_t B, uint32_t pitch, size_t codes_bytes, uint32_t want_cls,
                                                 const uint32_t* __restrict__ status,
                                                 double* __restrict__ lnl) {
  constexpr bool SWZ = NCOLS == 16;
  extern __shared__ __attribute__((aligned(16))) char smem[];
  double* tile = reinterpret_cast<double*>(smem);
  double* accs = tile + (size_t)TROWS * NCOLS;
  __shared__ uint32_t s_maxspan;
  const uint32_t gbeg = want_cls ? status[5] : 0, gend = want_cls ? status[4] : status[5];
  const uint32_t ng = gend - gbeg, ntiles = (B + NB - 1) / NB;
  const int t = threadIdx.x;
  for (uint32_t item = blockIdx.x; item < ng * ntiles; item += gridDim.x) {
  const Group g = groups[gbeg + item % ng];
  const uint32_t b0 = (item / ng) * NB;
  const uint32_t nb = min((uint32_t)NB, B - b0);
  __syncthreads();
  if (g.count == 0) continue;
  const bool active = t < (int)g.count;
  uint32_t qi = 0, begin = 0, span = 0;
  if (active) {
    qi = perm[g.start + t];
    begin = win_begin[qi];
    span = win_span[qi];
    if ((uint64_t)begin + span > W || (crel && span > cstride)) span = 0;
  }
  if (t == 0) s_maxspan = 0;
  __syncthreads();
  atomicMax(&s_maxspan, span);
  if (ACC) for (uint32_t j = 0; j < nb; ++j) accs[j * GQ + t] = 0.0;
  __syncthreads();
  const uint32_t gmin = win_begin[perm[g.start]];
  const uint32_t gspread = win_begin[perm[g.start + g.count - 1]] - gmin;
  const uint32_t rel = begin - gmin;
  const uint32_t nchunks = ACC ? (s_maxspan + CH - 1) / CH : 1;

  for (uint32_t c = 0; c < nchunks; ++c) {
    const uint32_t cbase = c * CH;
    const bool mine = active && cbase < span;
    const uint32_t rem = mine ? span - cbase : 0;
    uint32_t cw[CW];
    if (mine) {
      const size_t addr = (size_t)qi * cstride + (crel ? 0u : begin) + cbase;
      const size_t a0 = addr & ~(size_t)3;
      const uint32_t sh = (uint32_t)(addr & 3) * 8;
      const size_t last = (codes_bytes - 1) & ~(size_t)3;
      const uint32_t* p = reinterpret_cast<const uint32_t*>(codes);
      uint32_t prev = p[min(a0, last) >> 2];
#pragma unroll
      for (int i = 0; i < CW; ++i) {
        const uint32_t nxt = p[min(a0 + 4 * (i + 1), last) >> 2];
        const uint32_t v = __funnelshift_r(prev, nxt, sh);
        uint32_t o = v << 3;
        if (SWZ) {
          const uint32_t r = rel + 4 * i;
          o ^= (((r >> 1) & 15) << 3) | ((((r + 1) >> 1) & 15) << 11) | ((((r + 2) >> 1) & 15) << 19) |
               ((((r + 3) >> 1) & 15) << 27);
        }
        cw[i] = o;
        prev = nxt;
      }
    } else {
#pragma unroll
      for (int i = 0; i < CW; ++i) cw[i] = 0;
    }
    const uint32_t row0 = gmin + cbase;
    const uint32_t need = min((uint32_t)TROWS, gspread + min((uint32_t)CH, s_maxspan - cbase));
    for (uint32_t j = 0; j < nb; ++j) {
      __syncthreads();
      {
// ... 229 lines not shown
#define PP_XCD 1
#endif
using epa_wave::seg_key;
struct SegTrack {
  double m = -INFINITY;
  __device__ __forceinline__ void add(unsigned long long* __restrict__ segmax, uint32_t segp, uint32_t qi, uint32_t b,
                                      bool last, double v) {
    m = fmax(m, v);
    if ((b & 63u) == 63u || last) {
      atomicMax(&segmax[(size_t)qi * segp + (b >> 6)], seg_key(m));
      m = -INFINITY;
    }
  }
};

#ifndef PP_PRIO
#define PP_PRIO 1
#endif
template <int NBATCH>
__device__ __forceinline__ void gather_prio(int bt) {
#if PP_PRIO == 1
  if (bt == 0) __builtin_amdgcn_s_setprio(3);
  else if (bt == NBATCH / 4) __builtin_amdgcn_s_setprio(2);
  else if (bt == NBATCH / 2) __builtin_amdgcn_s_setprio(1);
  else if (bt == (3 * NBATCH) / 4) __builtin_amdgcn_s_setprio(0);
#elif PP_PRIO == 2
  if (bt == 0) __builtin_amdgcn_s_setprio(3);
  else if (bt == NBATCH / 2) __builtin_amdgcn_s_setprio(0);
#elif PP_PRIO == 3
  if (bt == 0) __builtin_amdgcn_s_setprio(3);
  else if (bt == (2 * NBATCH) / 5) __builtin_amdgcn_s_setprio(2);
  else if (bt == (7 * NBATCH) / 10) __builtin_amdgcn_s_setprio(1);
  else if (bt == (9 * NBATCH) / 10) __builtin_amdgcn_s_setprio(0);
#elif PP_PRIO == 4
  if (bt == 0) __builtin_amdgcn_s_setprio(3);
  else if (bt == NBATCH / 10) __builtin_amdgcn_s_setprio(2);
  else if (bt == (3 * NBATCH) / 10) __builtin_amdgcn_s_setprio(1);
  else if (bt == (6 * NBATCH) / 10) __builtin_amdgcn_s_setprio(0);
#endif
}

struct ItemWalk { uint32_t pos, end, step, lo; };
__device__ __forceinline__ ItemWalk item_walk(uint32_t total) {
  if (PP_XCD && (gridDim.x & 7u) == 0) {
    const uint32_t x = blockIdx.x & 7u, local = blockIdx.x >> 3;
    const uint32_t lo = (uint32_t)((uint64_t)total * x / 8), hi = (uint32_t)((uint64_t)total * (x + 1) / 8);
    return {lo + local, hi, gridDim.x >> 3, lo};
  }
  return {blockIdx.x, total, gridDim.x, 0u};
}

#ifndef PP_XCD_GROUPS
#define PP_XCD_GROUPS 1
#endif
__device__ __forceinline__ void item_group_tile(uint32_t v, uint32_t lo, uint32_t hi, uint32_t ng, uint32_t ntiles,
                                                uint32_t& grp, uint32_t& tile) {
  if (!PP_XCD_GROUPS) { grp = v % ng; tile = v / ng; return; }
  const uint32_t gl = lo / ntiles, tl = lo - gl * ntiles, gh = (hi - 1) / ntiles, th = (hi - 1) - gh * ntiles;
  uint32_t r = v - lo;
  for (uint32_t t = 0; t < ntiles; ++t) {
    const uint32_t first = gl + (t < tl ? 1u : 0u), last1 = gh + 1u - (t > th ? 1u : 0u);
    const uint32_t c = last1 > first ? last1 - first : 0u;
    if (r < c) { grp = first + r; tile = t; return; }
    r -= c;
  }
  grp = 0; tile = ntiles;
}

__device__ __forceinline__ uint32_t choose_tile(uint32_t ng, uint32_t B, uint32_t nwg) {
  uint32_t best = 32, best_cost = 0xffffffffu;
  for (uint32_t n = 16; n <= 96; n += 8) {
    const uint32_t items = ng * ((B + n - 1) / n);
    const uint32_t cost = ((items + nwg - 1) / nwg) * (n + 3);
    if (cost <= best_cost) { best_cost = cost; best = n; }
  }
  return best;
}

#ifdef PP_SCHED_PIN
#define PP_SCHED_BARRIER() __builtin_amdgcn_sched_barrier(0)
#else
#define PP_SCHED_BARRIER()
#endif
template <bool ACC, int SPR, int ROWL>
__global__ void __launch_bounds__(GQ2, 4) k_preplace_pairs(
    const double* __restrict__ lookup2, const uint16_t* __restrict__ packed,
    const uint16_t* __restrict__ tails, const uint32_t* __restrict__ win_begin,
    const uint32_t* __restrict__ win_span, const uint32_t* __restrict__ perm,
    const Group* __restrict__ groups, uint32_t W, uint32_t B, uint32_t pitch, uint32_t NP16,
    const uint32_t* __restrict__ status, double* __restrict__ lnl,
    unsigned long long* __restrict__ segmax, uint32_t segp) {
  constexpr int TR2 = (CH + SPR) / 2;
  extern __shared__ __attribute__((aligned(16))) char smem[];
  static_assert(ROWL % 16 == 0 && ROWL >= PROWB && ((TR2 - 1) * ROWL + PROWB) < 65536, "16-bit LDS offsets");
  double* accs = reinterpret_cast<double*>(smem + (size_t)TR2 * ROWL);
  __shared__ uint32_t s_maxspan;
  __shared__ uint32_t s_qi[GQ2];
  constexpr uint32_t BSTR = GQ2 + 4;
  const uint32_t ng = status[5];
  const uint32_t NBP = ACC ? NB2_ACC : choose_tile(ng, B, gridDim.x);
  const uint32_t ntiles = (B + NBP - 1) / NBP;
  const int t = threadIdx.x;
  const ItemWalk iw = item_walk(ng * ntiles);
  for (uint32_t item = iw.pos; item < iw.end; item += iw.step) {
  uint32_t item_g, item_t;
  item_group_tile(item, iw.lo, iw.end, ng, ntiles, item_g, item_t);
  const Group g = groups[item_g];
  const uint32_t b0 = item_t * NBP;
  const uint32_t nb = min(NBP, B - b0);
  __syncthreads();
  if (g.count == 0) continue;
  const bool active = t < (int)g.count;
  uint32_t qi = 0, begin = 0, span = 0;
  if (active) {
    qi = perm[g.start + t];
    begin = win_begin[qi];
    span = win_span[qi];
    if ((uint64_t)begin + span > W) span = 0;
  }
  if (t == 0) s_maxspan = 0;
  const uint32_t my_q = (active && span > 0) ? qi : 0xffffffffu;
  s_qi[t] = my_q;
  __syncthreads();
  {
    uint32_t m = span;
#pragma unroll
    for (int off = 32; off; off >>= 1) m = max(m, (uint32_t)__shfl_xor((int)m, off));
    if ((t & 63) == 0) atomicMax(&s_maxspan, m);
  }
  if (ACC) for (uint32_t j = 0; j < nb; ++j) accs[j * GQ2 + t] = 0.0;
  __syncthreads();
  const uint32_t gmin = win_begin[perm[g.start]];
  const uint32_t gspread = win_begin[perm[g.start + g.count - 1]] - gmin;
  const uint32_t rowoff = ((begin - gmin) >> 1) * ROWL;
  const uint32_t rowoff2 = rowoff | (rowoff << 16);
  const uint32_t nchunks = ACC ? (s_maxspan + CH - 1) / CH : 1;
  uint32_t t0 = 0, t1 = 0, t2 = 0, tailchunk = 0xffffffffu;
  if (active && (span & 3)) {
    const uint16_t* tq = tails + (size_t)qi * 4;
    t0 = tq[0] + rowoff; t1 = tq[1] + rowoff; t2 = tq[2] + rowoff;
    tailchunk = ((span >> 2) * 2) / CP;
  }
  auto at = [&](uint32_t off) -> double { return *reinterpret_cast<const double*>(smem + off); };
  SegTrack seg;

  for (uint32_t c = 0; c < nchunks; ++c) {
    const uint32_t cbase = c * CH;
    const bool mine = active && cbase < span;
    uint32_t cw[PW];
    if (mine) {
      const uint4* p = reinterpret_cast<const uint4*>(packed + (size_t)qi * NP16 + (size_t)c * CP);
#pragma unroll
      for (int i = 0; i < PW / 4; ++i) {
        const uint4 v = p[i];
        cw[4 * i] = v.x + rowoff2;
        cw[4 * i + 1] = v.y + rowoff2;
        cw[4 * i + 2] = v.z + rowoff2;
        cw[4 * i + 3] = v.w + rowoff2;
      }
    } else {
#pragma unroll
      for (int i = 0; i < PW; ++i) cw[i] = 0;
    }
    const uint32_t row0 = gmin + cbase;
    const uint32_t need = min((uint32_t)TR2, (gspread >> 1) + (min((uint32_t)CH, s_maxspan - cbase) + 1) / 2);
    const uint32_t rows = (row0 < W) ? min(need, (W - row0 + 1) / 2) : 0;
    const uint32_t n2 = rows * (PE / 2);
    constexpr int PF = (TR2 * (PE / 2) + GQ2 - 1) / GQ2;
    auto request = [&](uint32_t j, double2 (&pfs)[PF]) {
      const double2* src = reinterpret_cast<const double2*>(
          lookup2 + (((size_t)(b0 + j) * 2 + (row0 & 1u)) * ((W + 1) / 2) + (row0 >> 1)) * PE);
#pragma unroll
      for (int u = 0; u < PF; ++u) {
        const uint32_t i = u * GQ2 + t;
        pfs[u] = make_double2(0.0, 0.0);
        if (i < n2) pfs[u] = src[i];
      }
    };
    auto stage = [&](const double2 (&pfs)[PF], uint32_t boff) {
#pragma unroll
      for (int u = 0; u < PF; ++u) {
        const uint32_t i = u * GQ2 + t;
        if (i < n2) {
          if (ROWL == PROWB) {
            reinterpret_cast<double2*>(smem + boff)[i] = pfs[u];
          } else {
            const uint32_t r = i / (PE / 2), c2 = i - r * (PE / 2);
            *reinterpret_cast<double2*>(smem + boff + r * ROWL + c2 * 16) = pfs[u];
          }
        }
      }
// ... 4 lines not shown
#pragma unroll
        for (int i = 0; i < PW; ++i) asm volatile("" : "+v"(cw[i]));
#ifndef PP_WPB
#define PP_WPB 2
#endif
        constexpr int WPB = PP_WPB, NBATCH = PW / WPB;
        double rb[2][WPB * 2];
        auto issue = [&](int bt) {
#pragma unroll
          for (int w = 0; w < WPB; ++w) {
            const uint32_t v = cw[bt * WPB + w];
            rb[bt & 1][2 * w] = at((v & 0xffffu) + boff);
            rb[bt & 1][2 * w + 1] = at((v >> 16) + boff);
          }
        };
        issue(0);
        PP_SCHED_BARRIER();
#pragma unroll
        for (int bt = 0; bt < NBATCH; ++bt) {
          gather_prio<NBATCH>(bt);
          if (bt + 1 < NBATCH) issue(bt + 1);
          PP_SCHED_BARRIER();
#pragma unroll
          for (int w = 0; w < WPB; ++w) {
            const double s1 = rb[bt & 1][2 * w] + rb[bt & 1][2 * w + 1];
            sum += s1;
          }
          PP_SCHED_BARRIER();
        }
        if (c == tailchunk) {
          sum += at(t0 + boff);
          sum += at(t1 + boff);
          sum += at(t2 + boff);
        }
        if (ACC) {
          accs[j * GQ2 + t] = sum;
        } else {
          accs[(j & 7u) * BSTR + t] = sum;
          if (segmax) seg.add(segmax, segp, qi, b0 + j, j + 1 == nb, sum);
        }
      }
    };
    auto emit_burst = [&](uint32_t kb) {
      __builtin_amdgcn_wave_barrier();
      const uint32_t lane = (uint32_t)t & 63u, wbase = (uint32_t)t & ~63u, c4 = lane & 3u;
      const uint32_t ncol = min(8u, nb - 8u * kb), bcol = b0 + 8u * kb + 2u * c4;
      const uint32_t r0 = 2u * c4, r1 = 2u * c4 + 1u;
#pragma unroll
      for (uint32_t k = 0; k < 4; ++k) {
        const uint32_t tq = wbase + k * 16 + (lane >> 2);
        const uint32_t q = s_qi[tq];
        if (q != 0xffffffffu && 2u * c4 < ncol) {
          const double a0 = accs[r0 * BSTR + tq];
          double* dst = lnl + (size_t)q * pitch + bcol;
          if (2u * c4 + 1u < ncol) *reinterpret_cast<double2*>(dst) = make_double2(a0, accs[r1 * BSTR + tq]);
          else *dst = a0;
        }
      }
      __builtin_amdgcn_wave_barrier();
    };
    auto flush = [&](uint32_t j) {
      if (ACC) return;
      if ((j & 7u) == 7u) emit_burst(j >> 3);
      else if (j + 1 == nb) emit_burst(j >> 3);
    };
    {
      double2 pf[PF];
      request(0, pf);
      for (uint32_t j = 0; j < nb; ++j) {
        __syncthreads();
        stage(pf, 0);
        __syncthreads();
        if (j + 1 < nb) request(j + 1, pf);
        PP_SCHED_BARRIER();
        gather(j, 0);
        flush(j);
      }
    }
  }
  if (ACC && active) {
    double* out = lnl + (size_t)qi * pitch + b0;
    for (uint32_t j = 0; j < nb; ++j) out[j] = accs[j * GQ2 + t];
  }
  }
}

constexpr int CHS = 128;
constexpr int PWS = CHS / 2;
constexpr int TROWS_S = CHS + SPREAD;

template <int NCOLS>
__global__ void __launch_bounds__(256) k_pack_sites(const uint8_t* __restrict__ codes,
                                                    const uint32_t* __restrict__ win_begin,
                                                    const uint32_t* __restrict__ win_span, uint32_t Q,
                                                    uint32_t W, uint32_t cstride, uint32_t crel,
                                                    uint32_t span_bound, uint32_t NP16,
                                                    uint16_t* __restrict__ packed,
                                                    uint16_t* __restrict__ tails,
                                                    uint32_t* __restrict__ keys, uint32_t K,
                                                    uint32_t* __restrict__ status) {
  const uint32_t q = blockIdx.x * 4 + (threadIdx.x >> 6);
  const uint32_t lane = threadIdx.x & 63;
  if (q >= Q) return;
  const uint32_t begin = win_begin[q];
  uint32_t span = win_span[q];
  const uint32_t cmax = min(span_bound, crel ? cstride : 0xffffffffu);
  if (lane == 0) validate_window(q, begin, span, W, cmax, status);
  if ((uint64_t)begin + span > W || span > cmax) span = 0;
  const uint8_t* c = codes + (size_t)q * cstride + (crel ? 0u : begin);
  const uint32_t nsum = span & ~3u;
  for (uint32_t p = lane; p < NP16; p += 64) {
    uint32_t v = 0;
    if (p < nsum) v = (p % CHS) * (NCOLS * 8) + min((uint32_t)c[p], (uint32_t)NCOLS - 1) * 8;
    packed[(size_t)q * NP16 + p] = (uint16_t)v;
  }
  if (lane < 4) {
    uint32_t v = 0;
    if (lane < (span & 3))
      v = ((nsum + lane) % CHS) * (NCOLS * 8) + min((uint32_t)c[nsum + lane], (uint32_t)NCOLS - 1) * 8;
    tails[(size_t)q * 4 + lane] = (uint16_t)v;
  }
  if (lane == 0) {
    const uint32_t key = min(begin, K - 1);
    keys[q] = key;
  }
}

template <int NCOLS, bool ACC>
__global__ void __launch_bounds__(GQ2, 4) k_preplace_sites(
    const double* __restrict__ lookup, const uint16_t* __restrict__ packed,
    const uint16_t* __restrict__ tails, const uint32_t* __restrict__ win_begin,
    const uint32_t* __restrict__ win_span, const uint32_t* __restrict__ perm,
    const Group* __restrict__ groups, uint32_t W, uint32_t B, uint32_t pitch, uint32_t NP16,
    const uint32_t* __restrict__ status, double* __restrict__ lnl,
    unsigned long long* __restrict__ segmax, uint32_t segp) {
  constexpr uint32_t ROWB = NCOLS * 8;
  extern __shared__ __attribute__((aligned(16))) char smem[];
  double* accs = reinterpret_cast<double*>(smem + (size_t)TROWS_S * ROWB);
  __shared__ uint32_t s_maxspan;
  __shared__ uint32_t s_qi[GQ2];
  constexpr uint32_t BSTR = GQ2 + 4;
  const uint32_t ng = status[5];
  const uint32_t NBP = ACC ? NB2_ACC_S : choose_tile(ng, B, gridDim.x);
  const uint32_t ntiles = (B + NBP - 1) / NBP;
  const int t = threadIdx.x;
  auto at = [&](uint32_t off) -> double { return *reinterpret_cast<const double*>(smem + off); };
  const ItemWalk iw = item_walk(ng * ntiles);
  for (uint32_t item = iw.pos; item < iw.end; item += iw.step) {
    const Group g = groups[item % ng];
    const uint32_t b0 = (item / ng) * NBP;
    const uint32_t nb = min(NBP, B - b0);
    __syncthreads();
    SegTrack seg;
    if (g.count == 0) continue;
    const bool active = t < (int)g.count;
    uint32_t qi = 0, begin = 0, span = 0;
    if (active) {
      qi = perm[g.start + t];
      begin = win_begin[qi];
      span = win_span[qi];
      if ((uint64_t)begin + span > W) span = 0;
    }
    if (t == 0) s_maxspan = 0;
    s_qi[t] = (active && span > 0) ? qi : 0xffffffffu;
    __syncthreads();
    {
// ... 72 lines not shown
          double rb[2][WPB * 2];
          auto issue = [&](int bt) {
#pragma unroll
            for (int w = 0; w < WPB; ++w) {
              const uint32_t v = cw[bt * WPB + w];
              rb[bt & 1][2 * w] = at(v & 0xffffu);
              rb[bt & 1][2 * w + 1] = at(v >> 16);
            }
          };
          issue(0);
          __builtin_amdgcn_sched_barrier(0);
#pragma unroll
          for (int bt = 0; bt < NBATCH; ++bt) {
            gather_prio<NBATCH>(bt);
            if (bt + 1 < NBATCH) issue(bt + 1);
            __builtin_amdgcn_sched_barrier(0);
#pragma unroll
            for (int gq = 0; gq < 2; ++gq) {
              const double* v = &rb[bt & 1][gq * 4];
              double s1 = v[0] + v[1];
              const double s2 = v[2] + v[3];
              s1 += s2;
              sum += ((uint32_t)(bt * 2 + gq) < gfull) ? s1 : 0.0;
            }
            __builtin_amdgcn_sched_barrier(0);
          }
          if (c == tailchunk) {
            sum += at(t0);
            if (ntail > 1) sum += at(t1);
            if (ntail > 2) sum += at(t2);
          }
          if (ACC) {
            accs[j * GQ2 + t] = sum;
          } else {
            accs[(j & 7u) * BSTR + t] = sum;
            if (segmax) seg.add(segmax, segp, qi, b0 + j, j + 1 == nb, sum);
          }
        }
        if (!ACC && ((j & 7u) == 7u || j + 1 == nb)) {
          __builtin_amdgcn_wave_barrier();
          const uint32_t lane = (uint32_t)t & 63u, wbase = (uint32_t)t & ~63u, col = lane & 7u;
          const uint32_t ncol = (j & 7u) + 1u, bcol = b0 + (j & ~7u) + col;
#pragma unroll
          for (uint32_t k = 0; k < 8; ++k) {
            const uint32_t tq = wbase + k * 8 + (lane >> 3);
            const uint32_t q = s_qi[tq];
            if (q != 0xffffffffu && col < ncol) lnl[(size_t)q * pitch + bcol] = accs[col * BSTR + tq];
          }
          __builtin_amdgcn_wave_barrier();
        }
      }
    }
    if (ACC && active) {
      double* out = lnl + (size_t)qi * pitch + b0;
      for (uint32_t j = 0; j < nb; ++j) out[j] = accs[j * GQ2 + t];
    }
  }
}

}

void launch_scan_counts(epa_ctx* ctx, uint32_t* cnt, uint32_t K, const uint32_t* tip_row, uint32_t* tip_total) {
  hipLaunchKernelGGL(k_scan_counts, dim3(1), dim3(1024), 0, ctx->stream, cnt, K, tip_row, tip_total);
}

int launch_build_lookup2(epa_ctx* ctx) {
  if (!ctx->lookup2)
    EPA_HIP(ctx, hipMalloc(&ctx->lookup2, sizeof(double) * (size_t)ctx->B * 2 * ((ctx->W + 1) / 2) * PE));
  for (uint32_t b0 = 0; b0 < ctx->B; b0 += EPA_GRID_Y)
    hipLaunchKernelGGL(k_build_lookup2, dim3((ctx->W * PE + 255) / 256, std::min<uint32_t>(EPA_GRID_Y, ctx->B - b0)), dim3(256), 0,
                       ctx->stream, ctx->lookup, ctx->W, ctx->lookup2, b0);
  EPA_HIP(ctx, hipGetLastError());
  return EPA_OK;
}

int launch_build_lookup2_block(epa_ctx* ctx, uint32_t nb, const double* blk_lookup, double* blk_lookup2) {
  for (uint32_t r0 = 0; r0 < nb; r0 += EPA_GRID_Y)
    hipLaunchKernelGGL(k_build_lookup2, dim3((ctx->W * PE + 255) / 256, std::min<uint32_t>(EPA_GRID_Y, nb - r0)), dim3(256), 0,
                       ctx->stream, blk_lookup, ctx->W, blk_lookup2, r0);
  EPA_HIP(ctx, hipGetLastError());
  return EPA_OK;
}

int launch_preplace(epa_ctx* ctx, const uint8_t* d_codes, const uint32_t* d_begin, const uint32_t* d_span, uint32_t Q,
                    const PreTable& t, uint32_t max_span, const uint32_t** d_status) {
  double* const d_lnl = t.lnl;
  const uint32_t pitch = t.pitch, segp = t.segp;
  unsigned long long* const segmax = t.segmax;
  const bool blocked = ctx->lookup_blocks;
  const bool pairs = ctx->s == 4 && (ctx->lookup2 || blocked) && !ctx->opt.preplace_generic;
  const bool sites = ctx->s == 20 && ctx->ncols == 24 && !ctx->opt.preplace_generic;
  const uint32_t crel = ctx->code_stride ? 1u : 0u, cstride = crel ? ctx->code_stride : ctx->W;
  const uint32_t n_buckets = (ctx->W + SPREAD - 1) / SPREAD;
  const uint32_t Wp = n_buckets * SPREAD;
  const uint32_t n_blocks = pairs ? 4 : 1, class_blocks = pairs ? 2 : 1;
  const uint32_t gq0 = (pairs || sites) ? GQ2 : GQ, gq1 = GQ;
  const uint32_t max_runs = (Q + GQ - 1) / GQ + n_blocks;
  const uint32_t max_groups = max_runs + n_blocks * n_buckets;
  const uint32_t span_bound = (max_span == 0 || max_span > ctx->W) ? ctx->W : max_span;
  const uint32_t NP16 = pairs ? ((span_bound + 1) / 2 + CP - 1) / CP * CP
                        : sites ? (span_bound + CHS - 1) / CHS * CHS : 0;
  const uint32_t K = pairs ? n_blocks * Wp : sites ? ctx->W + 1 : 0;
  size_t temp_bytes = 0;
  (void)rocprim::radix_sort_pairs<epa_radix_cfg>(nullptr, temp_bytes, (uint32_t*)nullptr, (uint32_t*)nullptr,
                                  (uint32_t*)nullptr, (uint32_t*)nullptr, Q, 0, 32, ctx->stream);
  uint32_t *status, *key_cnt, *iota, *sorted_keys, *perm, *keys;
  Group* groups;
  uint16_t *packed, *tails;
  void* temp;
  auto layout = [&](Carver c) {
    status = c.take<uint32_t>(64);
    key_cnt = c.take<uint32_t>(K);
    iota = c.take<uint32_t>(Q);
    sorted_keys = c.take<uint32_t>(Q);
    perm = c.take<uint32_t>(Q);
    keys = c.take<uint32_t>(Q);
    groups = c.take<Group>(max_groups);
    packed = c.take<uint16_t>((size_t)Q * NP16);
    tails = c.take<uint16_t>((pairs || sites) ? 4 * (size_t)Q : 0);
    temp = c.tail(temp_bytes);
    return c.off;
  };
  char* base = (char*)epa_scratch(ctx, SLOT_PREPLACE, layout(Carver{}));
  if (!base) return epa_fail(ctx, EPA_ERR_HIP, "hipMalloc(preplace scratch)");
  layout(Carver{base});
  *d_status = status;
  {
    const int zr = epa_zero_async(ctx, status, (char*)iota - (char*)status, segmax, sizeof(unsigned long long) * (size_t)Q * segp);
    if (zr) return zr;
  }
  const bool acc = max_span == 0 || max_span > (uint32_t)CH;
  const bool wide = pairs && !acc && (uint64_t)Q * SPREAD < (uint64_t)1400 * ctx->W;
  const uint32_t rowl = (wide || acc) ? ROWL_PACKED : ROWL_NARROW;
  if (pairs) {
    constexpr uint32_t pack_grid = 64;
    hipLaunchKernelGGL(k_pack_pairs, dim3(std::min<uint32_t>((Q + 15) / 16, (uint32_t)ctx->n_cu * pack_grid)), dim3(256), 0, ctx->stream, d_codes, d_begin,
                       d_span, Q, ctx->W, cstride, crel, span_bound, Wp, NP16, rowl, packed, tails, keys, K, status);
  } else if (sites) {
    hipLaunchKernelGGL(k_pack_sites<24>, dim3((Q + 3) / 4), dim3(256), 0, ctx->stream, d_codes, d_begin,
                       d_span, Q, ctx->W, cstride, crel, span_bound, NP16, packed, tails, keys, K, status);
  }
  if (pairs || sites) {
    hipLaunchKernelGGL(k_count_keys, dim3((Q + 255) / 256), dim3(256), 0, ctx->stream, keys, Q, key_cnt, iota);
    launch_scan_counts(ctx, key_cnt, K);
    hipLaunchKernelGGL(k_scatter_sorted, dim3((Q + 255) / 256), dim3(256), 0, ctx->stream, keys, iota, key_cnt, Q,
                       sorted_keys, perm);
  } else {
    hipLaunchKernelGGL(k_iota, dim3((Q + 255) / 256), dim3(256), 0, ctx->stream, iota, Q);
    hipLaunchKernelGGL(k_validate, dim3((Q + 255) / 256), dim3(256), 0, ctx->stream, d_begin, d_span, Q,
                       ctx->W, std::min(span_bound, crel ? cstride : 0xffffffffu), status);
    int wbits = 1;
    while (wbits < 32 && (1ull << wbits) <= (uint64_t)ctx->W) ++wbits;
    EPA_HIP(ctx, rocprim::radix_sort_pairs<epa_radix_cfg>(temp, temp_bytes, d_begin, sorted_keys, iota, perm, Q, 0, wbits,
                                           ctx->stream));
  }
  constexpr int SPREAD_WIDE = 288;
  hipLaunchKernelGGL(k_make_groups, dim3(1), dim3(256),
                     sizeof(uint32_t) * (2 * (n_blocks + 1) + 4 * (size_t)max_runs + 2), ctx->stream,
                     sorted_keys, Q, pairs ? Wp : 0xffffffffu, n_blocks, class_blocks, gq0, gq1,
                     (uint32_t)(wide ? SPREAD_WIDE : SPREAD), max_runs, groups, max_groups, status);
  const size_t codes_bytes = (size_t)Q * cstride;
  const uint32_t want_cls = pairs ? 1u : 0u;
  const size_t lds = sizeof(double) * ((size_t)TROWS * ctx->ncols + (acc ? (size_t)NB * GQ : 0));
  const size_t lds2 = wide ? (size_t)((CH + SPREAD_WIDE) / 2) * ROWL_PACKED + sizeof(double) * NB2_BURST * (GQ2 + 4)
                           : (size_t)TROWS2 * rowl + sizeof(double) * (acc ? NB2_ACC * GQ2 : NB2_BURST * (GQ2 + 4));
  const bool acc_s = max_span == 0 || max_span > (uint32_t)CHS;
  const size_t lds_s = (size_t)TROWS_S * 24 * 8 + sizeof(double) * (acc_s ? NB2_ACC_S * GQ2 : NB2_BURST * (GQ2 + 4));
  using FastKernel = decltype(&k_preplace_sites<24, false>);
  using GenericKernel = decltype(&k_preplace<16, false>);
  FastKernel k_fast = nullptr;
  if (pairs) k_fast = wide ? k_preplace_pairs<false, SPREAD_WIDE, ROWL_PACKED> : acc ? k_preplace_pairs<true, SPREAD, ROWL_PACKED> : k_preplace_pairs<false, SPREAD, ROWL_NARROW>;
  else if (sites) k_fast = acc_s ? k_preplace_sites<24, true> : k_preplace_sites<24, false>;
  const bool fast_acc = pairs ? acc : acc_s;
  const size_t lds_fast = pairs ? lds2 : lds_s;
  const GenericKernel k_generic = sites ? nullptr : ctx->ncols == 16 ? (acc ? k_preplace<16, true> : k_preplace<16, false>) : (acc ? k_preplace<24, true> : k_preplace<24, false>);
  if (k_fast) EPA_HIP(ctx, hipFuncSetAttribute((const void*)k_fast, hipFuncAttributeMaxDynamicSharedMemorySize, (int)lds_fast));
  if (k_generic) EPA_HIP(ctx, hipFuncSetAttribute((const void*)k_generic, hipFuncAttributeMaxDynamicSharedMemorySize, (int)lds));
  auto kernels = [&](const double* lk, const double* lk2, uint32_t nB, double* lnl, unsigned long long* sm) {
    if (k_fast) {
      const uint32_t tile = fast_acc ? (pairs ? NB2_ACC : NB2_ACC_S) : 16;
      const dim3 grid_f((uint32_t)std::min<uint64_t>((uint64_t)max_groups * ((nB + tile - 1) / tile), (uint64_t)ctx->n_cu));
      hipLaunchKernelGGL(k_fast, grid_f, dim3(GQ2), (uint32_t)lds_fast, ctx->stream, pairs ? lk2 : lk, (const uint16_t*)packed,
                         (const uint16_t*)tails, d_begin, d_span, perm, groups, ctx->W, nB, pitch, NP16, status, lnl,
                         fast_acc ? nullptr : sm, segp);
    }
    if (!k_generic) return;
    const uint32_t ntiles = (nB + NB - 1) / NB;
    const dim3 grid(pairs ? (uint32_t)std::min<uint64_t>((uint64_t)max_groups * ntiles, (uint64_t)ctx->n_cu * (acc ? 2 : 4))
                          : max_groups * ntiles);
    hipLaunchKernelGGL(k_generic, grid, dim3(GQ), (uint32_t)lds, ctx->stream, lk, d_codes, d_begin, d_span, perm, groups, ctx->W,
                       cstride, crel, nB, pitch, codes_bytes, want_cls, status, lnl);
  };
  if (!blocked) {
    epa_timer_start(ctx, epa_t(ctx, epa_ctx::T_PREPLACE));
    kernels(ctx->lookup, ctx->lookup2, ctx->B, d_lnl, segmax);
    epa_timer_stop(ctx, epa_t(ctx, epa_ctx::T_PREPLACE));
    EPA_HIP(ctx, hipGetLastError());
    return EPA_OK;
  }
  const uint32_t blk = epa_block_branches(ctx);
  size_t off2 = 0;
  (void)epa_block_bytes(ctx->s, ctx->W, blk, &off2);
  char* buf = (char*)epa_block_buffer(ctx);
  if (!buf) return epa_fail(ctx, EPA_ERR_NO_MEMORY, "hipMalloc(lookup block buffer): " + std::to_string(epa_block_bytes(ctx->s, ctx->W, blk, nullptr)) +
                                                    " bytes needed for blocks of " + std::to_string(blk) + " branches (option lookup_block)");
  double* blk_lookup = reinterpret_cast<double*>(buf);
  double* blk_lookup2 = ctx->s == 4 ? reinterpret_cast<double*>(buf + off2) : nullptr;
  const uint32_t nblocks = (ctx->B + blk - 1) / blk;
  std::vector<hipEvent_t>& ev = ctx->blk_ev[ctx->bank];
  const bool timed = ctx->opt.timers != 0;
  ctx->blk_ev_n[ctx->bank] = 0;
  (void)epa_t(ctx, epa_ctx::T_PREPLACE);
  auto mark = [&](uint32_t i) -> int {
    if (!timed) return EPA_OK;
    while (ev.size() <= i) { hipEvent_t e = nullptr; EPA_HIP(ctx, hipEventCreate(&e)); ev.push_back(e); }
    EPA_HIP(ctx, hipEventRecord(ev[i], ctx->stream));
    return EPA_OK;
  };
  for (uint32_t k = 0; k < nblocks; ++k) {
    const uint32_t b0 = k * blk, nB = std::min(blk, ctx->B - b0);
    int rc = mark(2 * k);
    if (!rc) rc = launch_build_lookup_block(ctx, b0, nB, blk_lookup);
    if (!rc && pairs) rc = launch_build_lookup2_block(ctx, nB, blk_lookup, blk_lookup2);
    if (!rc) rc = mark(2 * k + 1);
    if (rc) return rc;
    kernels(blk_lookup, blk_lookup2, nB, d_lnl + b0, segmax ? segmax + (b0 >> 6) : nullptr);
  }
  { const int rc = mark(2 * nblocks); if (rc) return rc; }
  if (timed) ctx->blk_ev_n[ctx->bank] = 2 * nblocks + 1;
  EPA_HIP(ctx, hipGetLastError());
  return EPA_OK;
}

int preplace_window_error(epa_ctx* ctx, const uint32_t* st) {
  if (st[0])
    return epa_fail(ctx, EPA_ERR_QUERY_ALL_GAP, "Sequence " + std::to_string(st[0] & 0x7fffffffu) +
                                                    " does not appear to have any non-gap sites!");
  if (st[1])
    return epa_fail(ctx, EPA_ERR_QUERY_WIDTH, "Query sequence length not same as reference alignment!");
  return EPA_OK;
}

int preplace_check_status(epa_ctx* ctx, const uint32_t* d_status) {
  uint32_t st[4];
  EPA_HIP(ctx, hipMemcpy(st, d_status, sizeof(st), hipMemcpyDeviceToHost));
  return preplace_window_error(ctx, st);
}
```

### epa_ng_amd/csrc/select.hip

```cpp
#include "epa_dev_internal.hpp"
#include "wave_util.hpp"

#include <rocprim/device/device_scan.hpp>

#include <algorithm>
#include <cmath>

namespace {

using epa_wave::seg_key;
using epa_wave::seg_val;


struct SelOut {
  unsigned long long* stage;
  uint32_t cap;
  uint32_t* bitmap;
  uint32_t* bcount;
  uint32_t wpr;
  __device__ __forceinline__ void put(uint32_t q, uint32_t bi, uint32_t taken, uint32_t* status) const {
    if (bitmap) {
      atomicOr(&bitmap[(size_t)bi * wpr + (q >> 5)], 1u << (q & 31u));
      atomicAdd(&bcount[bi], 1u);
    } else if (taken < cap) {
// ... 517 lines not shown
  if (t < RB_WORDS - RB_WINDOW) out[RB_WINDOW + t] = pre_status ? pre_status[t] : 0u;
  __syncthreads();
  if (tip_total && t == 0) {
    int one = -1, n = 0;
    for (int c = 0; c < EPA_N_CLS; ++c)
      if (status[SEL_HIST + c]) { one = c; ++n; }
    if (n == 1 && epa_tip_class_ok(one)) {
      const uint32_t all = status[SEL_HIST + one], tips = min(*tip_total, all);
      out[RB_HIST + one] = all - tips;
      out[RB_HIST + epa_tip_class(one)] = tips;
      out[RB_TIP_SPLIT] = 1u;
    }
  }
}

__global__ void __launch_bounds__(256) k_compact(const unsigned long long* __restrict__ stage,
                                                 const uint32_t* __restrict__ counts,
                                                 const uint32_t* __restrict__ offsets, uint32_t Q,
                                                 uint32_t cap, unsigned long long* __restrict__ keys) {
  const uint32_t q = blockIdx.x * 4 + (threadIdx.x >> 6);
  const int lane = threadIdx.x & 63;
  if (q >= Q) return;
  const uint32_t n = counts[q], o = offsets[q];
  for (uint32_t i = lane; i < n; i += 64) keys[o + i] = stage[(size_t)q * cap + i];
}

__global__ void __launch_bounds__(256) k_emit_pairs(const uint32_t* __restrict__ bitmap, uint32_t wpr,
                                                    const uint32_t* __restrict__ boffs,
                                                    epa_pair* __restrict__ pairs, uint32_t nb, uint32_t max_pairs) {
  __shared__ uint32_t wsum[4];
  const uint32_t b = blockIdx.x, t = threadIdx.x, lane = t & 63u, wv = t >> 6;
  if (boffs[nb] > max_pairs) return;
  uint32_t base = boffs[b];
  const uint32_t end = boffs[b + 1];
  if (base == end) return;
  const uint32_t* row = bitmap + (size_t)b * wpr;
  for (uint32_t w0 = 0; w0 < wpr && base < end; w0 += 256) {
    const uint32_t wi = w0 + t;
    uint32_t bits = wi < wpr ? row[wi] : 0u;
    const uint32_t c = (uint32_t)__popc(bits);
    uint32_t inc = c;
#pragma unroll
    for (int o = 1; o < 64; o <<= 1) {
      const uint32_t u = __shfl_up(inc, o);
      if ((int)lane >= o) inc += u;
    }
    if (lane == 63) wsum[wv] = inc;
    __syncthreads();
    uint32_t before = 0, total = 0;
#pragma unroll
    for (uint32_t w = 0; w < 4; ++w) {
      if (w < wv) before += wsum[w];
      total += wsum[w];
    }
    uint32_t o = base + before + inc - c;
    while (bits) {
      const uint32_t k = (uint32_t)__ffs((int)bits) - 1u;
      bits &= bits - 1u;
      pairs[o].branch_id = b;
      pairs[o].seq_id = wi * 32u + k;
      ++o;
    }
    base += total;
    __syncthreads();
  }
}

__global__ void k_keys_to_pairs(const unsigned long long* __restrict__ keys, uint64_t n,
                                epa_pair* __restrict__ pairs) {
  const uint64_t i = (uint64_t)blockIdx.x * blockDim.x + threadIdx.x;
  if (i < n) {
    pairs[i].branch_id = (uint32_t)(keys[i] >> 32);
    pairs[i].seq_id = (uint32_t)(keys[i] & 0xffffffffu);
  }
}

void emit_pairs(epa_ctx* ctx, const SelectPending* sp) {
  hipLaunchKernelGGL(k_emit_pairs, dim3(ctx->B), dim3(256), 0, ctx->stream, sp->bitmap, sp->wpr, sp->boffs, sp->d_pairs, ctx->B,
                     (uint32_t)std::min<uint64_t>(sp->max_pairs, 0xffffffffu));
}

}

int launch_select_begin(epa_ctx* ctx, const PreTable& t, const uint32_t* pre_status, uint32_t Q, double threshold,
                        epa_pair* d_pairs, uint64_t max_pairs, const uint32_t* d_span, uint32_t* rb, SelectPending* sp) {
  sp->have_hist = false;
  const uint32_t B = ctx->B;
  const double* const d_lnl = t.lnl;
  const uint32_t pitch = t.pitch;
  const int mode = ctx->heur_mode;
  uint32_t limit = 0;
  if (mode == 1) {
    limit = (uint32_t)std::min<double>((double)B, std::ceil(ctx->heur_param * (double)B));
    ctx->select_cap = std::max(ctx->select_cap, std::max(limit, 1u));
  } else if (mode == 2) {
    ctx->select_cap = std::max(ctx->select_cap, std::min(B, 48u));
  }
  const uint32_t cap = ctx->select_cap;
  size_t scan_bytes = 0, sort_bytes = 0;
  (void)rocprim::exclusive_scan(nullptr, scan_bytes, (uint32_t*)nullptr, (uint32_t*)nullptr, 0u, Q,
                                rocprim::plus<uint32_t>(), ctx->stream);
  const size_t worst = std::min<uint64_t>(max_pairs, (uint64_t)Q * cap);
  (void)rocprim::radix_sort_keys<epa_radix_cfg>(nullptr, sort_bytes, (unsigned long long*)nullptr,
                                 (unsigned long long*)nullptr, worst, 0, 64, ctx->stream);
  const uint32_t wpr = (Q + 31) / 32;
  const bool bm = !ctx->opt.select_sort && (size_t)B * wpr * sizeof(uint32_t) <= ((size_t)64 << 20);
  uint32_t* status = nullptr;
  size_t fill = 0;
  auto layout = [&](Carver c) {
    status = c.take<uint32_t>(SEL_WORDS);
    if (bm) {
      sp->boffs = c.take<uint32_t>((size_t)B + 1);
      sp->bitmap = c.take<uint32_t>((size_t)B * wpr);
      fill = c.off;
      sp->counts = c.take<uint32_t>(Q + 1);
    } else {
      sp->counts = c.take<uint32_t>(Q + 1);
      sp->offsets = c.take<uint32_t>(Q + 1);
      sp->stage = c.take<unsigned long long>((size_t)Q * cap);
      sp->keys_a = c.take<unsigned long long>(worst);
      sp->keys_b = c.take<unsigned long long>(worst);
      sp->temp = c.tail(std::max(scan_bytes, sort_bytes));
    }
    return c.off;
  };
  char* base = (char*)epa_scratch(ctx, SLOT_SELECT, layout(Carver{}));
  if (!base) return epa_fail(ctx, EPA_ERR_HIP, "hipMalloc(select scratch)");
  sp->bitmap = nullptr; sp->offsets = nullptr;
  layout(Carver{base});
  uint32_t* const counts = sp->counts;
  sp->wpr = wpr; sp->sort_bytes = sort_bytes;
  sp->table = t; sp->pre_status = pre_status; sp->Q = Q; sp->threshold = threshold; sp->d_pairs = d_pairs; sp->max_pairs = max_pairs;
  sp->d_span = d_span; sp->cap = cap; sp->rb = rb;
  sp->ev_rb = nullptr; sp->d_rb = nullptr; sp->emitted = false; sp->queued_cls = -1;
  if (bm) {
    const int zr = epa_zero_async(ctx, base, fill);
    if (zr) return zr;
  } else {
    EPA_HIP(ctx, hipMemsetAsync(status, 0, sizeof(uint32_t) * SEL_WORDS, ctx->stream));
    EPA_HIP(ctx, hipMemsetAsync(counts + Q, 0, sizeof(uint32_t), ctx->stream));
  }
  epa_timer_start(ctx, epa_t(ctx, epa_ctx::T_SELECT));
  auto select_rows = [&](const SelOut& so) -> bool {
    const int nr = (int)((B + 63) / 64);
    if (so.bitmap && t.segmax && !ctx->opt.select_full_rows && mode == 0 && threshold < 1.0 && nr <= 64) {
      const double band_x = 1.0 - std::log((1.0 - threshold) / (double)B);
      const double band_t = std::max(band_x, std::log((double)B) + 38.0);
      constexpr uint32_t sel_grid = 16;
      const dim3 grid_seg(std::min<uint32_t>((Q + 3) / 4, (uint32_t)ctx->n_cu * sel_grid));
      hipLaunchKernelGGL(k_select_seg<8>, grid_seg, dim3(256), 0, ctx->stream, d_lnl, t.segmax, t.segp, Q, B, pitch, threshold,
                         band_x, band_t, so, counts, status, d_span, ctx->s, d_span ? status + SEL_HIST : nullptr);
      return d_span != nullptr;
    }
    auto rows = [&](auto kernel, dim3 grid) {
      hipLaunchKernelGGL(kernel, grid, dim3(256), 0, ctx->stream, d_lnl, Q, B, pitch, threshold, mode, limit, so, counts, status);
    };
    const dim3 waves((Q + 3) / 4);
    if (nr <= 2) rows(k_select<2>, waves); else if (nr <= 4) rows(k_select<4>, waves); else if (nr <= 8) rows(k_select<8>, waves);
    else if (nr <= 16) rows(k_select<16>, waves); else if (nr <= 32) rows(k_select<32>, waves); else if (nr <= 64) rows(k_select<64>, waves);
    else if (nr <= 128) rows(k_select_wg<32>, dim3(Q)); else if (nr <= 256) rows(k_select_wg<64>, dim3(Q));
    else {
      const double stream_band = (mode == 0 && threshold > 0.0 && threshold < 1.0) ? 1.0 - std::log((1.0 - threshold) / (double)B) : 0.0;
      hipLaunchKernelGGL(k_select_stream, dim3(Q), dim3(256), 0, ctx->stream, d_lnl, Q, B, pitch, threshold, stream_band, mode, limit, so, counts, status);
    }
    return false;
  };
  const bool seg_hist = select_rows(bm ? SelOut{nullptr, 0u, sp->bitmap, sp->boffs, wpr} : SelOut{sp->stage, cap, nullptr, nullptr, 0u});
  uint32_t* const tip_total = (bm && epa_tipd_active(ctx) && d_span) ? status + SEL_TIP_TOTAL : nullptr;
  const uint32_t* total;
  if (bm) {
    launch_scan_counts(ctx, sp->boffs, B + 1, tip_total ? ctx->tip_row : nullptr, tip_total);
    total = sp->boffs + B;
  } else {
    EPA_HIP(ctx, rocprim::exclusive_scan(sp->temp, scan_bytes, counts, sp->offsets, 0u, Q + 1, rocprim::plus<uint32_t>(), ctx->stream));
    total = sp->offsets + Q;
  }
  if (d_span && !seg_hist)
    hipLaunchKernelGGL(k_class_hist, dim3((Q + 255) / 256), dim3(256), 0, ctx->stream, counts, d_span, Q, ctx->s, status + SEL_HIST);
  hipLaunchKernelGGL(k_pack_readback, dim3(1), dim3(64), 0, ctx->stream, status, total, sp->pre_status, status + SEL_READBACK,
                     (const uint32_t*)tip_total);
  EPA_HIP(ctx, hipMemcpyAsync(rb, status + SEL_READBACK, sizeof(uint32_t) * RB_WORDS, hipMemcpyDeviceToHost, ctx->stream));
  sp->have_status = sp->pre_status != nullptr;
  if (bm) {
    if (!ctx->ev_rb[ctx->bank]) EPA_HIP(ctx, hipEventCreateWithFlags(&ctx->ev_rb[ctx->bank], hipEventDisableTiming));
    EPA_HIP(ctx, hipEventRecord(ctx->ev_rb[ctx->bank], ctx->stream));
    sp->ev_rb = ctx->ev_rb[ctx->bank];
    sp->d_rb = status + SEL_READBACK;
  }
  return EPA_OK;
}

int launch_select_emit(epa_ctx* ctx, SelectPending* sp) {
  if (!sp->bitmap || !sp->d_rb || sp->emitted) return EPA_OK;
  emit_pairs(ctx, sp);
  epa_timer_stop(ctx, epa_t(ctx, epa_ctx::T_SELECT));
  EPA_HIP(ctx, hipGetLastError());
  sp->emitted = true;
  return EPA_OK;
}

int launch_select_end(epa_ctx* ctx, SelectPending* sp, uint64_t* n_pairs) {
  const uint32_t B = ctx->B, Q = sp->Q;
  for (;;) {
    if (sp->ev_rb) EPA_HIP(ctx, hipEventSynchronize(sp->ev_rb));
    else EPA_HIP(ctx, hipStreamSynchronize(ctx->stream));
    const uint32_t total = sp->rb[RB_TOTAL];
    const uint32_t overflow = sp->rb[RB_STATUS + SEL_OVERFLOW];
    if (overflow && !sp->bitmap) {
      if (sp->cap >= B) return epa_fail(ctx, EPA_ERR_HIP, "select_candidates: staging overflow");
      ctx->select_cap = std::min<uint32_t>(B, std::max(sp->cap * 4, overflow));
      int rc = launch_select_begin(ctx, sp->table, sp->pre_status, Q, sp->threshold, sp->d_pairs, sp->max_pairs, sp->d_span, sp->rb, sp);
      if (rc) return rc;
      continue;
    }
    if (total > sp->max_pairs)
      return epa_fail(ctx, EPA_ERR_PAIR_OVERFLOW,
                      "select_candidates: " + std::to_string(total) + " candidates exceed max_pairs");
    if (total && sp->bitmap) {
      if (!sp->emitted) emit_pairs(ctx, sp);
    } else if (total) {
      const dim3 grid((Q + 3) / 4);
      hipLaunchKernelGGL(k_compact, grid, dim3(256), 0, ctx->stream, sp->stage, sp->counts, sp->offsets, Q, sp->cap,
                         sp->keys_a);
      int bits = 33;
      while ((1ull << (bits - 32)) <= B && bits < 64) ++bits;
      size_t sort_bytes = sp->sort_bytes;
      EPA_HIP(ctx, rocprim::radix_sort_keys<epa_radix_cfg>(sp->temp, sort_bytes, sp->keys_a, sp->keys_b, (size_t)total,
                                                           32, bits, ctx->stream));
      hipLaunchKernelGGL(k_keys_to_pairs, dim3((total + 255) / 256), dim3(256), 0, ctx->stream, sp->keys_b,
                         (uint64_t)total, sp->d_pairs);
// ... 27 lines not shown
```

### include/epa_dev.h

```cpp
#ifndef EPA_DEV_H
#define EPA_DEV_H

#include <stddef.h>
#include <stdint.h>

#ifdef __cplusplus
extern "C" {
#endif

typedef struct epa_ctx epa_ctx;

typedef enum {
  EPA_OK = 0,
  EPA_ERR_INVALID_ARG = -1,
  EPA_ERR_HIP = -2,
  EPA_ERR_NO_DEVICE = -3,
  EPA_ERR_QUERY_WIDTH = -4,
  EPA_ERR_QUERY_ALL_GAP = -5,
  EPA_ERR_INVALID_CHAR = -6,
  EPA_ERR_NEG_INF = -7,
  EPA_ERR_UNSUPPORTED = -8,
  EPA_ERR_PAIR_OVERFLOW = -9,
  EPA_ERR_NO_MEMORY = -10
} epa_status;
// ... 55 lines not shown
  const double* rec_length_a;
  const double* rec_length_b;
  const uint32_t* branch_prox;
  const uint32_t* branch_dist;
} epa_tree_desc;

typedef struct {
  uint32_t branch_id;
  uint32_t seq_id;
} epa_pair;

typedef struct {
  double lnl;
  double pendant_length;
  double distal_length;
} epa_result;

typedef struct {
  uint64_t pairs;
  uint64_t rounds;
  uint64_t newton_evals;
  uint64_t reverts;
} epa_thorough_stats;

int epa_dev_device_count(void);

int epa_dev_create(const epa_ref_desc* desc, int device, epa_ctx** out);
void epa_dev_destroy(epa_ctx* ctx);
const char* epa_dev_last_error(const epa_ctx* ctx);

int epa_dev_create_from_tree(const epa_tree_desc* tree, int device, epa_ctx** out);

int epa_dev_tree_logl(epa_ctx* ctx, uint32_t branch, double* lnl);

int epa_dev_set_stream(epa_ctx* ctx, void* hip_stream);

int epa_dev_set_option(epa_ctx* ctx, const char* key, int value);

int epa_dev_build_lookup(epa_ctx* ctx);

typedef struct {
  uint64_t reft;
  uint64_t scsum;
  uint64_t lookup;
  uint64_t lookup2;
  uint64_t refi;
  uint64_t misc;
  uint64_t create_temp;
  uint64_t reference;
  uint64_t bank;
  uint64_t steady;
  uint64_t peak;
} epa_footprint;
int epa_dev_footprint(uint32_t states, uint32_t rate_cats, uint64_t sites, uint64_t branches, int flags, int from_tree,
                      uint32_t block_branches, int banks, epa_footprint* out);

#define EPA_LOOKUP_RESIDENT 0
#define EPA_LOOKUP_BLOCKS 1
int epa_dev_lookup_plan(uint64_t usable_bytes, uint32_t states, uint32_t rate_cats, uint64_t sites, uint64_t branches,
                        int flags, int from_tree, int banks, int* mode, uint32_t* block_branches);
void epa_dev_set_mem_cap(uint64_t bytes);
int epa_dev_lookup_mode(const epa_ctx* ctx, int* mode, uint32_t* block_branches);


int epa_encode_queries(uint32_t states, uint32_t sites, uint32_t Q, const char* const* seqs,
                       int premasking, int aa_x_as_n, uint8_t* codes, uint32_t* win_begin,
                       uint32_t* win_span, uint32_t* bad_query);

void epa_encode_set_threads(unsigned n);
int epa_encode_queries_compact(uint32_t states, uint32_t sites, uint32_t Q, const char* const* seqs,
                               int premasking, int aa_x_as_n, uint32_t stride, uint8_t* codes,
                               uint32_t* win_begin, uint32_t* win_span, uint32_t* bad_query);
int epa_dev_set_query_layout(epa_ctx* ctx, uint32_t code_stride);

int epa_pack_codes_4bit(const uint8_t* codes, uint32_t Q, uint32_t stride, uint8_t* packed);
int epa_unpack_codes_4bit(const uint8_t* packed, uint32_t Q, uint32_t stride, uint8_t* codes);
int epa_dev_set_query_packing(epa_ctx* ctx, int bits);

int epa_dev_preplace(epa_ctx* ctx, const uint8_t* q_codes, const uint32_t* win_begin,
                     const uint32_t* win_span, uint32_t Q, double* lnl);

int epa_dev_preplace_bounded(epa_ctx* ctx, const uint8_t* q_codes, const uint32_t* win_begin,
                             const uint32_t* win_span, uint32_t Q, uint32_t max_span, double* lnl, uint64_t* seg_keys);

int epa_dev_thorough(epa_ctx* ctx, const epa_pair* pairs, uint64_t n_pairs,
                     const uint8_t* q_codes, const uint32_t* win_begin, const uint32_t* win_span,
                     uint32_t Q, epa_result* out, epa_thorough_stats* stats);

int epa_dev_score_at(epa_ctx* ctx, const epa_pair* pairs, const double* pendant, const double* distal,
                     const double* proximal , uint64_t n,
                     const uint8_t* q_codes, const uint32_t* win_begin, const uint32_t* win_span, uint32_t Q,
                     double* lnl);

int epa_dev_site_lnl(epa_ctx* ctx, const epa_pair* pairs, const double* pendant, const double* distal,
                     const double* proximal , uint64_t n,
                     const uint8_t* q_codes, const uint32_t* win_begin, const uint32_t* win_span, uint32_t Q,
                     uint32_t pitch, double* site_lnl );

int epa_dev_preplace_profile(epa_ctx* ctx, const double* prof, uint32_t stride, const uint32_t* win_begin,
                             const uint32_t* win_span, uint32_t Q, double* lnl);
int epa_dev_thorough_profile(epa_ctx* ctx, const epa_pair* pairs, uint64_t n_pairs, const double* prof, uint32_t stride,
                             const uint32_t* win_begin, const uint32_t* win_span, uint32_t Q, epa_result* out,
                             epa_thorough_stats* stats);
int epa_dev_score_at_profile(epa_ctx* ctx, const epa_pair* pairs, const double* pendant, const double* distal,
                             const double* proximal , uint64_t n, const double* prof, uint32_t stride,
                             const uint32_t* win_begin, const uint32_t* win_span, uint32_t Q, double* lnl);
int epa_dev_site_lnl_profile(epa_ctx* ctx, const epa_pair* pairs, const double* pendant, const double* distal,
                             const double* proximal , uint64_t n, const double* prof, uint32_t stride,
                             const uint32_t* win_begin, const uint32_t* win_span, uint32_t Q, uint32_t pitch,
                             double* site_lnl );
int epa_dev_place_chunk_profile(epa_ctx* ctx, const double* prof, uint32_t stride, const uint32_t* win_begin,
                                const uint32_t* win_span, uint32_t Q, double threshold, epa_pair* pairs,
                                epa_result* results, uint64_t max_pairs, uint64_t* n_pairs, epa_thorough_stats* stats);
int epa_profile_from_phred(uint32_t states, uint32_t Q, uint32_t stride, const uint8_t* codes, const uint8_t* phred,
                           const uint32_t* win_span, double* prof);

int epa_dev_marginal_like(epa_ctx* ctx, const epa_pair* pairs, uint64_t n,
                          const double* x_frac, const double* x_logw, uint32_t Kx,
                          const double* p_len,  const double* p_logw, uint32_t Kp,
                          const uint8_t* q_codes, const uint32_t* win_begin, const uint32_t* win_span, uint32_t Q,
                          double* marginal , double* grid_lnl );

int epa_quadrature_legendre01(uint32_t K, double* nodes, double* log_weights);
int epa_quadrature_laguerre(uint32_t K, double* nodes, double* log_weights);

int epa_dev_rell_support(epa_ctx* ctx, const epa_pair* pairs, const double* pendant, const double* distal,
                         const double* proximal , uint64_t n,
                         const uint8_t* q_codes, const uint32_t* win_begin, const uint32_t* win_span, uint32_t Q,
                         const uint64_t* stream_id ,
                         uint32_t replicates, uint64_t seed, double* support );

int epa_dev_rell_tests(epa_ctx* ctx, const epa_pair* pairs, const double* pendant, const double* distal,
                       const double* proximal , uint64_t n,
                       const uint8_t* q_codes, const uint32_t* win_begin, const uint32_t* win_span, uint32_t Q,
                       const uint64_t* stream_id ,
                       uint32_t replicates, uint64_t seed,
                       double* support , double* elw , double* p_sh );

int epa_dev_rell_au(epa_ctx* ctx, const epa_pair* pairs, const double* pendant, const double* distal,
                    const double* proximal , uint64_t n,
                    const uint8_t* q_codes, const uint32_t* win_begin, const uint32_t* win_span, uint32_t Q,
                    const uint64_t* stream_id ,
                    uint32_t replicates, uint64_t seed,
                    const uint32_t* scale_pm , uint32_t n_scales,
                    double* p_au , uint32_t* counts ,
                    double* fit );

int epa_dev_rell_kh(epa_ctx* ctx, const epa_pair* pairs, const double* pendant, const double* distal,
                    const double* proximal , uint64_t n,
                    const uint8_t* q_codes, const uint32_t* win_begin, const uint32_t* win_span, uint32_t Q,
                    const uint64_t* stream_id ,
                    uint32_t replicates, uint64_t seed,
                    double* p_kh , double* p_wkh , double* p_wsh );

int epa_dev_select_candidates(epa_ctx* ctx, const double* lnl, uint32_t Q, double threshold,
                              epa_pair* pairs, uint64_t max_pairs, uint64_t* n_pairs);

#define EPA_HEUR_DYNAMIC 0
#define EPA_HEUR_FIXED 1
#define EPA_HEUR_BASEBALL 2
int epa_dev_set_heuristic(epa_ctx* ctx, int mode, double param);

int epa_dev_place_chunk(epa_ctx* ctx, const uint8_t* q_codes, const uint32_t* win_begin,
                        const uint32_t* win_span, uint32_t Q, uint32_t max_span, double threshold,
                        epa_pair* pairs, epa_result* results, uint64_t max_pairs,
                        uint64_t* n_pairs, epa_thorough_stats* stats);
// ... 77 lines not shown
```

Before: 17.60 million placements/s.

## Screen preplacement with fp32 lookup and recompute only candidate segments in fp64

Adds a float32 copy of the pair lookup table and a screening preplace kernel that scores every branch pair in fp32 and records per-segment maxima. A band kernel uses an error bound (delta) and the selection band to mark which 64-branch segments can hold candidates. Only those segments are regrouped and recomputed exactly in fp64 with a sparse variant of the pairs kernel. The aim is to skip most fp64 preplacement work, at the cost of extra kernels, scratch memory, and reliance on the fp32 error bound being conservative enough to keep selection correct. A probe API is also added for inspection.

```diff
diff --git a/epa_ng_amd/api.py b/epa_ng_amd/api.py
--- a/epa_ng_amd/api.py
+++ b/epa_ng_amd/api.py
@@ -96,6 +96,10 @@
                                        C.c_void_p]
         L.epa_dev_preplace_bounded.argtypes = [C.c_void_p, C.c_void_p, C.c_void_p, C.c_void_p, C.c_uint32, C.c_uint32,
                                                C.c_void_p, C.c_void_p]
+        L.epa_dev_preplace_screen_probe.argtypes = [C.c_void_p, C.c_void_p, C.c_void_p, C.c_void_p, C.c_uint32, C.c_uint32,
+                                                    C.c_double, C.c_void_p, C.c_void_p, C.c_void_p]
+        L.epa_dev_preplace_screen_runs.argtypes = [C.c_void_p]
+        L.epa_dev_preplace_screen_runs.restype = C.c_uint64
         L.epa_dev_thorough.argtypes = [C.c_void_p, C.c_void_p, C.c_uint64, C.c_void_p, C.c_void_p,
                                        C.c_void_p, C.c_uint32, C.c_void_p, C.POINTER(_Stats)]
         L.epa_dev_score_at.argtypes = [C.c_void_p, C.c_void_p, C.c_void_p, C.c_void_p, C.c_void_p, C.c_uint64,
@@ -451,6 +455,23 @@
                                                     int(max_span), _ptr(out), _ptr(keys)))
         return (out, keys) if seg_keys else out
 
+    def preplace_screen_runs(self):
+        return int(self.L.epa_dev_preplace_screen_runs(self.h))
+
+    def preplace_screen_probe(self, codes, win_begin, win_span, max_span, threshold=0.99999, arrays=True):
+        Q = len(win_begin)
+        nseg = (self.B + 63) // 64
+        seg32 = np.full((Q, nseg), np.nan, np.float32) if arrays else None
+        mask = np.zeros(Q, np.uint64) if arrays else None
+        info = np.zeros(8, np.float64)
+        self._layout(codes)
+        self._check(self.L.epa_dev_preplace_screen_probe(self.h, _ptr(codes), _ptr(win_begin), _ptr(win_span), Q,
+                                                         int(max_span), float(threshold), _ptr(seg32), _ptr(mask),
+                                                         _ptr(info)))
+        return {"ran": bool(info[0]), "delta": float(info[1]), "included": int(info[2]), "M": float(info[3]),
+                "nonfinite": int(info[4]), "band_t": float(info[5]), "ms_screen": float(info[6]),
+                "ms_band": float(info[7]), "seg32": seg32, "mask": mask}
+
     def thorough(self, pairs, codes, win_begin, win_span, Q=None, n_pairs=None, out=None):
         Q = len(win_begin) if Q is None else Q
         n = len(pairs) if n_pairs is None else n_pairs
diff --git a/epa_ng_amd/csrc/chunk.hip b/epa_ng_amd/csrc/chunk.hip
--- a/epa_ng_amd/csrc/chunk.hip
+++ b/epa_ng_amd/csrc/chunk.hip
@@ -17,6 +17,7 @@
     t.segmax = (unsigned long long*)epa_scratch(ctx, SLOT_SEGMAX, sizeof(unsigned long long) * (size_t)Q * t.segp);
     if (!t.segmax) return epa_fail(ctx, EPA_ERR_HIP, "hipMalloc(segment maxima)");
   }
+  if (epa_select_takes_seg(ctx, t, Q, threshold)) t.band_t = epa_select_band_t(threshold, ctx->B);
   const uint32_t* pre_status = nullptr;
   int rc = launch_preplace(ctx, d_codes, d_begin, d_span, Q, t, max_span, &pre_status);
   if (!rc) rc = launch_select_begin(ctx, t, pre_status, Q, threshold, d_pairs, max_pairs, d_span, rb, sp);
diff --git a/epa_ng_amd/csrc/epa_dev.hip b/epa_ng_amd/csrc/epa_dev.hip
--- a/epa_ng_amd/csrc/epa_dev.hip
+++ b/epa_ng_amd/csrc/epa_dev.hip
@@ -587,7 +587,8 @@
       {"select_full_rows", &EpaOptions::select_full_rows}, {"select_sort", &EpaOptions::select_sort},
       {"queued_thorough", &EpaOptions::queued_thorough},   {"xcd_balance", &EpaOptions::xcd_balance},
       {"aa_valu", &EpaOptions::aa_valu},                   {"timers", &EpaOptions::timers},
-      {"newton_lds", &EpaOptions::newton_lds},             {"tip_distal", &EpaOptions::tip_distal}};
+      {"newton_lds", &EpaOptions::newton_lds},             {"tip_distal", &EpaOptions::tip_distal},
+      {"preplace_screen", &EpaOptions::preplace_screen},   {"preplace_screen_scale", &EpaOptions::preplace_screen_scale}};
   for (const Entry& e : table)
     if (strcmp(key, e.name) == 0) {
       ctx->opt.*e.field = value;
@@ -676,6 +677,7 @@
   if (ctx->blen) (void)hipFree(ctx->blen);
   if (ctx->lookup) (void)hipFree(ctx->lookup);
   if (ctx->lookup2) (void)hipFree(ctx->lookup2);
+  if (ctx->lookup2f) (void)hipFree(ctx->lookup2f);
   if (ctx->prof_tab) (void)hipFree(ctx->prof_tab);
   for (void* p : ctx->blk_buf) if (p) (void)hipFree(p);
   for (auto& v : ctx->blk_ev) for (hipEvent_t e : v) if (e) (void)hipEventDestroy(e);
@@ -1521,6 +1523,61 @@
                                 epa_is_device_ptr(seg_keys) ? hipMemcpyDeviceToDevice : hipMemcpyDeviceToHost, ctx->stream));
   EPA_HIP(ctx, hipStreamSynchronize(ctx->stream));
   return preplace_check_status(ctx, d_status);
+}
+
+extern "C" uint64_t epa_dev_preplace_screen_runs(const epa_ctx* ctx) { return ctx ? ctx->screen_runs : 0; }
+
+extern "C" int epa_dev_preplace_screen_probe(epa_ctx* ctx, const uint8_t* q_codes, const uint32_t* win_begin,
+                                             const uint32_t* win_span, uint32_t Q, uint32_t max_span, double threshold,
+                                             float* seg32, uint64_t* seg_mask, double* info) {
+  if (!ctx || !q_codes || !win_begin || !win_span || !info)
+    return epa_fail(ctx, EPA_ERR_INVALID_ARG, "null argument");
+  for (int i = 0; i < 8; ++i) info[i] = 0.0;
+  if (Q == 0) return EPA_OK;
+  EPA_HIP(ctx, hipSetDevice(ctx->device));
+  int rc = epa_dev_build_lookup(ctx);
+  if (rc) return rc;
+  if (max_span > ctx->W) max_span = ctx->W;
+  if (max_span && !epa_is_device_ptr(win_span))
+    for (uint32_t q = 0; q < Q; ++q)
+      if (win_span[q] > max_span) return epa_fail(ctx, EPA_ERR_INVALID_ARG, "preplace: a window is longer than max_span");
+  if (ctx->s == 4 && ctx->lookup2 && (rc = launch_build_lookup2f(ctx))) return rc;
+  const uint8_t* d_codes = epa_codes_to_device(ctx, q_codes, Q);
+  const uint32_t* d_begin = (const uint32_t*)epa_to_device(ctx, SLOT_BEGIN, win_begin, sizeof(uint32_t) * Q);
+  const uint32_t* d_span = (const uint32_t*)epa_to_device(ctx, SLOT_SPAN, win_span, sizeof(uint32_t) * Q);
+  if (!d_codes || !d_begin || !d_span) return epa_fail(ctx, EPA_ERR_HIP, "query upload failed");
+  PreScreenProbe probe;
+  probe.band_t = epa_select_band_t(threshold, ctx->B);
+  const uint32_t* d_status = nullptr;
+  rc = launch_preplace(ctx, d_codes, d_begin, d_span, Q, PreTable{}, max_span, &d_status, &probe);
+  if (rc) return rc;
+  EPA_HIP(ctx, hipStreamSynchronize(ctx->stream));
+  if ((rc = preplace_check_status(ctx, d_status))) return rc;
+  info[0] = probe.ran ? 1.0 : 0.0;
+  info[3] = ctx->screen_M;
+  info[4] = (double)ctx->screen_nonfinite;
+  info[5] = probe.band_t;
+  if (!probe.ran) return EPA_OK;
+  const uint32_t nseg = (ctx->B + 63) / 64, segp = (nseg + 7u) & ~7u;
+  unsigned long long n_incl = 0;
+  EPA_HIP(ctx, hipMemcpy(&n_incl, probe.n_incl, sizeof(n_incl), hipMemcpyDeviceToHost));
+  info[1] = probe.delta;
+  info[2] = (double)n_incl;
+  info[6] = probe.ms_screen;
+  info[7] = probe.ms_band;
+  if (seg_mask) EPA_HIP(ctx, hipMemcpy(seg_mask, probe.mask, sizeof(uint64_t) * Q, hipMemcpyDeviceToHost));
+  if (seg32) {
+    std::vector<uint32_t> keys((size_t)Q * segp);
+    EPA_HIP(ctx, hipMemcpy(keys.data(), probe.seg32, sizeof(uint32_t) * keys.size(), hipMemcpyDeviceToHost));
+    for (uint32_t q = 0; q < Q; ++q)
+      for (uint32_t s = 0; s < nseg; ++s) {
+        const uint32_t k = keys[(size_t)q * segp + s], u = (k >> 31) ? (k & 0x7fffffffu) : ~k;
+        float v = NAN;
+        if (k) memcpy(&v, &u, 4);
+        seg32[(size_t)q * nseg + s] = v;
+      }
+  }
+  return EPA_OK;
 }
 
 extern "C" int epa_dev_thorough(epa_ctx* ctx, const epa_pair* pairs, uint64_t n_pairs,
diff --git a/epa_ng_amd/csrc/epa_dev_internal.hpp b/epa_ng_amd/csrc/epa_dev_internal.hpp
--- a/epa_ng_amd/csrc/epa_dev_internal.hpp
+++ b/epa_ng_amd/csrc/epa_dev_internal.hpp
@@ -3,6 +3,8 @@
 #include <hip/hip_runtime.h>
 #include <stdint.h>
 
+#include <algorithm>
+#include <cmath>
 #include <string>
 #include <vector>
 
@@ -83,7 +85,15 @@
   uint32_t pitch = 0;
   unsigned long long* segmax = nullptr;
   uint32_t segp = 0;
-};
+  double band_t = 0.0;
+};
+
+inline double epa_select_band_x(double threshold, uint32_t B) { return 1.0 - std::log((1.0 - threshold) / (double)B); }
+inline double epa_select_band_t(double threshold, uint32_t B) {
+  return std::max(epa_select_band_x(threshold, B), std::log((double)B) + 38.0);
+}
+
+bool epa_select_takes_seg(const epa_ctx* ctx, const PreTable& t, uint32_t Q, double threshold);
 
 struct SelectPending {
   PreTable table;
@@ -229,6 +239,8 @@
   int newton_lds = 0;
   int tip_distal = 1;
   int dedup_key_bits = 64;
+  int preplace_screen = 1;
+  int preplace_screen_scale = 1;
   int dedup_sort_bits = 32;
 };
 
@@ -262,6 +274,11 @@
   double* cinv = nullptr;
   double inv_w0 = 0.0;
   double* lookup2 = nullptr;
+  float2* lookup2f = nullptr;
+  bool lookup2f_refused = false;
+  uint64_t screen_runs = 0;
+  double screen_M = 0.0;
+  uint64_t screen_nonfinite = 0;
   uint32_t* tip_row = nullptr;
   uint8_t* tipmask = nullptr;
   double* tipd = nullptr;
@@ -418,13 +435,24 @@
                      const uint32_t* d_tipmap, uint32_t tipmap_size, double* dst);
 int launch_build_lookup(epa_ctx* ctx);
 int launch_build_lookup2(epa_ctx* ctx);
+int launch_build_lookup2f(epa_ctx* ctx);
+double epa_screen_delta(const epa_ctx* ctx, uint32_t span_bound);
+struct PreScreenProbe {
+  double band_t = 0.0;
+  bool ran = false;
+  double delta = 0.0;
+  const uint32_t* seg32 = nullptr;
+  const unsigned long long* mask = nullptr;
+  const unsigned long long* n_incl = nullptr;
+  float ms_screen = -1.f, ms_band = -1.f;
+};
 uint32_t epa_block_branches(const epa_ctx* ctx);
 size_t epa_block_bytes(int s, uint32_t W, uint32_t blk, size_t* off2);
 void* epa_block_buffer(epa_ctx* ctx);
 int launch_build_lookup_block(epa_ctx* ctx, uint32_t b0, uint32_t nb, double* blk_lookup);
 int launch_build_lookup2_block(epa_ctx* ctx, uint32_t nb, const double* blk_lookup, double* blk_lookup2);
 int launch_preplace(epa_ctx* ctx, const uint8_t* d_codes, const uint32_t* d_begin, const uint32_t* d_span, uint32_t Q,
-                    const PreTable& t, uint32_t max_span, const uint32_t** d_status);
+                    const PreTable& t, uint32_t max_span, const uint32_t** d_status, PreScreenProbe* probe = nullptr);
 int preplace_check_status(epa_ctx* ctx, const uint32_t* d_status);
 __attribute__((visibility("hidden"))) int preplace_window_error(epa_ctx* ctx, const uint32_t* st);
 __attribute__((visibility("hidden"))) void launch_scan_counts(epa_ctx* ctx, uint32_t* cnt, uint32_t K, const uint32_t* tip_row = nullptr,
diff --git a/epa_ng_amd/csrc/preplace.hip b/epa_ng_amd/csrc/preplace.hip
--- a/epa_ng_amd/csrc/preplace.hip
+++ b/epa_ng_amd/csrc/preplace.hip
@@ -106,8 +106,10 @@
                                                      uint32_t Wp, uint32_t n_blocks,
                                                      uint32_t class_blocks, uint32_t gq0, uint32_t gq1,
                                                      uint32_t spr0, uint32_t max_runs, Group* __restrict__ groups,
-                                                     uint32_t max_groups, uint32_t* __restrict__ status) {
+                                                     uint32_t max_groups, uint32_t* __restrict__ status,
+                                                     const uint32_t* __restrict__ n_dev = nullptr, uint32_t seg_div = 0) {
   extern __shared__ uint32_t sh[];
+  if (n_dev) Q = min(Q, *n_dev);
   uint32_t* lo = sh;
   uint32_t* runbase = lo + n_blocks + 1;
   uint32_t* run_start = runbase + n_blocks + 1;
@@ -167,14 +169,14 @@
     const uint32_t cls = b >= class_blocks ? 1u : 0u;
     const uint32_t start = run_start[r], end = run_end[r], g0 = run_off[r], n = run_off[r + 1] - g0;
     if (n == 1) {
-      if (g0 < max_groups) groups[g0] = Group{start, end - start, 0, cls};
+      if (g0 < max_groups) groups[g0] = Group{start, end - start, seg_div ? sorted_keys[start] / seg_div : 0u, cls};
     } else {
       const uint32_t spr = cls ? (uint32_t)SPREAD : spr0;
       const uint32_t kb = sorted_keys[start] / spr;
       uint32_t a = start;
       for (uint32_t k = 0; k < n; ++k) {
         const uint32_t e = k + 1 == n ? end : lower_bound(a, end, (uint64_t)(kb + k + 1) * spr);
-        if (g0 + k < max_groups) groups[g0 + k] = Group{a, e - a, 0, cls};
+        if (g0 + k < max_groups) groups[g0 + k] = Group{a, e - a, (seg_div && e > a) ? sorted_keys[a] / seg_div : 0u, cls};
         a = e;
       }
     }
@@ -570,7 +572,7 @@
 #else
 #define PP_SCHED_BARRIER()
 #endif
-template <bool ACC, int SPR, int ROWL>
+template <bool ACC, int SPR, int ROWL, bool SPARSE = false>
 __global__ void __launch_bounds__(GQ2, 4) k_preplace_pairs(
     const double* __restrict__ lookup2, const uint16_t* __restrict__ packed,
     const uint16_t* __restrict__ tails, const uint32_t* __restrict__ win_begin,
@@ -586,15 +588,15 @@
   __shared__ uint32_t s_qi[GQ2];
   constexpr uint32_t BSTR = GQ2 + 4;
   const uint32_t ng = status[5];
-  const uint32_t NBP = ACC ? NB2_ACC : choose_tile(ng, B, gridDim.x);
-  const uint32_t ntiles = (B + NBP - 1) / NBP;
+  const uint32_t NBP = SPARSE ? 64u : ACC ? NB2_ACC : choose_tile(ng, B, gridDim.x);
+  const uint32_t ntiles = SPARSE ? 1u : (B + NBP - 1) / NBP;
   const int t = threadIdx.x;
-  const ItemWalk iw = item_walk(ng * ntiles);
+  const ItemWalk iw = SPARSE ? ItemWalk{blockIdx.x, ng, gridDim.x, 0u} : item_walk(ng * ntiles);
   for (uint32_t item = iw.pos; item < iw.end; item += iw.step) {
-  uint32_t item_g, item_t;
-  item_group_tile(item, iw.lo, iw.end, ng, ntiles, item_g, item_t);
+  uint32_t item_g = item, item_t = 0;
+  if (!SPARSE) item_group_tile(item, iw.lo, iw.end, ng, ntiles, item_g, item_t);
   const Group g = groups[item_g];
-  const uint32_t b0 = item_t * NBP;
+  const uint32_t b0 = SPARSE ? min(g.min_begin * 64u, B - 1u) : item_t * NBP;
   const uint32_t nb = min(NBP, B - b0);
   __syncthreads();
   if (g.count == 0) continue;
@@ -765,6 +767,252 @@
     double* out = lnl + (size_t)qi * pitch + b0;
     for (uint32_t j = 0; j < nb; ++j) out[j] = accs[j * GQ2 + t];
   }
+  }
+}
+
+typedef float f2 __attribute__((ext_vector_type(2)));
+
+__device__ __forceinline__ uint32_t seg_key32(float v) {
+  const uint32_t u = __float_as_uint(v);
+  return (u >> 31) ? ~u : (u | 0x80000000u);
+}
+__device__ __forceinline__ float seg_val32(uint32_t k) { return __uint_as_float((k >> 31) ? (k & 0x7fffffffu) : ~k); }
+
+__global__ void __launch_bounds__(256) k_build_lookup2f(const double* __restrict__ lookup2, uint32_t W, uint32_t B,
+                                                        float2* __restrict__ lookup2f, uint32_t p0,
+                                                        uint32_t* __restrict__ stats) {
+  const uint32_t p = p0 + blockIdx.y, Wh = (W + 1) / 2, n = 2 * Wh * PE;
+  const uint32_t i = blockIdx.x * 256 + threadIdx.x;
+  float amax = 0.f;
+  uint32_t bad = 0;
+  if (i < n) {
+    const uint32_t par = i / (Wh * PE), rem = i - par * Wh * PE, r = rem / PE, e = rem - r * PE;
+    const bool valid = 2 * r + par < W, two = 2 * p + 1 < B;
+    float x = 0.f, y = 0.f;
+    if (valid) {
+      x = (float)lookup2[(size_t)(2 * p) * n + i];
+      y = two ? (float)lookup2[(size_t)(2 * p + 1) * n + i] : (e == PE - 1 ? 0.f : -INFINITY);
+      const bool fx = isfinite(x), fy = !two || isfinite(y);
+      bad = (fx ? 0u : 1u) + (fy ? 0u : 1u);
+      if (fx) amax = fabsf(x);
+      if (two && fy) amax = fmaxf(amax, fabsf(y));
+    }
+    lookup2f[(size_t)p * n + i] = make_float2(x, y);
+  }
+#pragma unroll
+  for (int off = 32; off; off >>= 1) {
+    amax = fmaxf(amax, __shfl_xor(amax, off));
+    bad += (uint32_t)__shfl_xor((int)bad, off);
+  }
+  if ((threadIdx.x & 63) == 0) {
+    if (amax > 0.f) atomicMax(&stats[0], __float_as_uint(amax));
+    if (bad) atomicAdd(&stats[1], bad);
+  }
+}
+
+template <int SPR, int ROWL>
+__global__ void __launch_bounds__(GQ2, 4) k_preplace_screen(
+    const float2* __restrict__ lookup2f, const uint16_t* __restrict__ packed,
+    const uint16_t* __restrict__ tails, const uint32_t* __restrict__ win_begin,
+    const uint32_t* __restrict__ win_span, const uint32_t* __restrict__ perm,
+    const Group* __restrict__ groups, uint32_t W, uint32_t BP, uint32_t NP16,
+    const uint32_t* __restrict__ status, uint32_t* __restrict__ seg32, uint32_t segp) {
+  constexpr int TR2 = (CH + SPR) / 2;
+  extern __shared__ __attribute__((aligned(16))) char smem[];
+  static_assert(ROWL % 16 == 0 && ROWL >= PROWB && ((TR2 - 1) * ROWL + PROWB) < 65536, "16-bit LDS offsets");
+  __shared__ uint32_t s_maxspan;
+  const uint32_t ng = status[5];
+  const uint32_t NBP = choose_tile(ng, BP, gridDim.x);
+  const uint32_t ntiles = (BP + NBP - 1) / NBP;
+  const int t = threadIdx.x;
+  const ItemWalk iw = item_walk(ng * ntiles);
+  for (uint32_t item = iw.pos; item < iw.end; item += iw.step) {
+    uint32_t item_g, item_t;
+    item_group_tile(item, iw.lo, iw.end, ng, ntiles, item_g, item_t);
+    const Group g = groups[item_g];
+    const uint32_t b0 = item_t * NBP;
+    const uint32_t nb = min(NBP, BP - b0);
+    __syncthreads();
+    if (g.count == 0) continue;
+    const bool active = t < (int)g.count;
+    uint32_t qi = 0, begin = 0, span = 0;
+    if (active) {
+      qi = perm[g.start + t];
+      begin = win_begin[qi];
+      span = win_span[qi];
+      if ((uint64_t)begin + span > W) span = 0;
+    }
+    if (t == 0) s_maxspan = 0;
+    __syncthreads();
+    {
+      uint32_t m = span;
+#pragma unroll
+      for (int off = 32; off; off >>= 1) m = max(m, (uint32_t)__shfl_xor((int)m, off));
+      if ((t & 63) == 0) atomicMax(&s_maxspan, m);
+    }
+    __syncthreads();
+    const uint32_t gmin = win_begin[perm[g.start]];
+    const uint32_t gspread = win_begin[perm[g.start + g.count - 1]] - gmin;
+    const uint32_t rowoff = ((begin - gmin) >> 1) * ROWL;
+    const uint32_t rowoff2 = rowoff | (rowoff << 16);
+    const bool mine = active && span > 0;
+    uint32_t t0 = 0, t1 = 0, t2 = 0;
+    if (mine && (span & 3)) {
+      const uint16_t* tq = tails + (size_t)qi * 4;
+      t0 = tq[0] + rowoff; t1 = tq[1] + rowoff; t2 = tq[2] + rowoff;
+    }
+    auto at = [&](uint32_t off) -> f2 { return *reinterpret_cast<const f2*>(smem + off); };
+    uint32_t cw[PW];
+    if (mine) {
+      const uint4* p = reinterpret_cast<const uint4*>(packed + (size_t)qi * NP16);
+#pragma unroll
+      for (int i = 0; i < PW / 4; ++i) {
+        const uint4 v = p[i];
+        cw[4 * i] = v.x + rowoff2;
+        cw[4 * i + 1] = v.y + rowoff2;
+        cw[4 * i + 2] = v.z + rowoff2;
+        cw[4 * i + 3] = v.w + rowoff2;
+      }
+    } else {
+#pragma unroll
+      for (int i = 0; i < PW; ++i) cw[i] = 0;
+    }
+    const uint32_t row0 = gmin;
+    const uint32_t need = min((uint32_t)TR2, (gspread >> 1) + (min((uint32_t)CH, s_maxspan) + 1) / 2);
+    const uint32_t rows = (row0 < W) ? min(need, (W - row0 + 1) / 2) : 0;
+    const uint32_t n2 = rows * (PE / 2);
+    constexpr int PF = (TR2 * (PE / 2) + GQ2 - 1) / GQ2;
+    auto request = [&](uint32_t j, float4 (&pfs)[PF]) {
+      const float4* src = reinterpret_cast<const float4*>(
+          lookup2f + (((size_t)(b0 + j) * 2 + (row0 & 1u)) * ((W + 1) / 2) + (row0 >> 1)) * PE);
+#pragma unroll
+      for (int u = 0; u < PF; ++u) {
+        const uint32_t i = u * GQ2 + t;
+        pfs[u] = make_float4(0.f, 0.f, 0.f, 0.f);
+        if (i < n2) pfs[u] = src[i];
+      }
+    };
+    auto stage = [&](const float4 (&pfs)[PF]) {
+#pragma unroll
+      for (int u = 0; u < PF; ++u) {
+        const uint32_t i = u * GQ2 + t;
+        if (i < n2) {
+          if (ROWL == PROWB) {
+            reinterpret_cast<float4*>(smem)[i] = pfs[u];
+          } else {
+            const uint32_t r = i / (PE / 2), c2 = i - r * (PE / 2);
+            *reinterpret_cast<float4*>(smem + r * ROWL + c2 * 16) = pfs[u];
+          }
+        }
+      }
+    };
+    float segm = -INFINITY;
+    auto gather = [&](uint32_t j) {
+      if (!mine) return;
+      f2 sum = {0.f, 0.f};
+#pragma unroll
+      for (int i = 0; i < PW; ++i) asm volatile("" : "+v"(cw[i]));
+      constexpr int WPB = PP_WPB, NBATCH = PW / WPB;
+      f2 rb[2][WPB * 2];
+      auto issue = [&](int bt) {
+#pragma unroll
+        for (int w = 0; w < WPB; ++w) {
+          const uint32_t v = cw[bt * WPB + w];
+          rb[bt & 1][2 * w] = at(v & 0xffffu);
+          rb[bt & 1][2 * w + 1] = at(v >> 16);
+        }
+      };
+      issue(0);
+#pragma unroll
+      for (int bt = 0; bt < NBATCH; ++bt) {
+        gather_prio<NBATCH>(bt);
+        if (bt + 1 < NBATCH) issue(bt + 1);
+#pragma unroll
+        for (int w = 0; w < WPB; ++w) {
+          const f2 s1 = rb[bt & 1][2 * w] + rb[bt & 1][2 * w + 1];
+          sum += s1;
+        }
+      }
+      if (span & 3) {
+        sum += at(t0);
+        sum += at(t1);
+        sum += at(t2);
+      }
+      segm = fmaxf(segm, fmaxf(sum.x, sum.y));
+      const uint32_t bp = b0 + j;
+      if ((bp & 31u) == 31u || j + 1 == nb) {
+        atomicMax(&seg32[(size_t)qi * segp + (bp >> 5)], seg_key32(segm));
+        segm = -INFINITY;
+      }
+    };
+    float4 pf[PF];
+    request(0, pf);
+    for (uint32_t j = 0; j < nb; ++j) {
+      __syncthreads();
+      stage(pf);
+      __syncthreads();
+      if (j + 1 < nb) request(j + 1, pf);
+      gather(j);
+    }
+  }
+}
+
+__global__ void __launch_bounds__(256) k_screen_band(const uint32_t* __restrict__ seg32, uint32_t Q, uint32_t nseg,
+                                                     uint32_t seg32p, double band, double delta,
+                                                     const uint32_t* __restrict__ qkeys, uint32_t KB,
+                                                     unsigned long long* __restrict__ segmax, uint32_t segp,
+                                                     uint32_t* __restrict__ ccnt, uint32_t* __restrict__ rank,
+                                                     unsigned long long* __restrict__ mask,
+                                                     unsigned long long* __restrict__ n_incl) {
+  const uint32_t q = blockIdx.x * 256 + threadIdx.x;
+  uint32_t cnt = 0;
+  if (q < Q) {
+    const uint32_t* row = seg32 + (size_t)q * seg32p;
+    const uint32_t qk = qkeys[q];
+    float r = -INFINITY;
+    bool all = qk < KB;
+    for (uint32_t s = 0; s < nseg; ++s) {
+      const uint32_t k = row[s];
+      if (k) r = fmaxf(r, seg_val32(k)); else all = false;
+    }
+    unsigned long long m = 0;
+    if (all) {
+      const double lo = (double)r - band;
+      for (uint32_t s = 0; s < nseg; ++s) {
+        const double v = (double)seg_val32(row[s]);
+        if (v >= lo) {
+          m |= 1ull << s;
+          if (ccnt) rank[(size_t)q * seg32p + s] = atomicAdd(&ccnt[s * KB + qk], 1u);
+        } else if (segmax) {
+          segmax[(size_t)q * segp + s] = seg_key(v + delta);
+        }
+      }
+    }
+    mask[q] = m;
+    cnt = (uint32_t)__popcll(m);
+  }
+#pragma unroll
+  for (int off = 32; off; off >>= 1) cnt += (uint32_t)__shfl_xor((int)cnt, off);
+  if ((threadIdx.x & 63) == 0 && cnt) atomicAdd(n_incl, (unsigned long long)cnt);
+}
+
+__global__ void __launch_bounds__(256) k_scatter_cells(const unsigned long long* __restrict__ mask,
+                                                       const uint32_t* __restrict__ qkeys, const uint32_t* __restrict__ rank,
+                                                       const uint32_t* __restrict__ offs, uint32_t Q, uint32_t seg32p,
+                                                       uint32_t KB, uint32_t ncell, uint32_t* __restrict__ sorted_keys,
+                                                       uint32_t* __restrict__ perm) {
+  const uint32_t q = blockIdx.x * 256 + threadIdx.x;
+  if (q >= Q) return;
+  unsigned long long m = mask[q];
+  const uint32_t qk = qkeys[q];
+  while (m) {
+    const uint32_t s = (uint32_t)__ffsll((long long)m) - 1u;
+    m &= m - 1;
+    const uint32_t key = s * KB + qk, pos = offs[key] + rank[(size_t)q * seg32p + s];
+    if (pos < ncell) {
+      sorted_keys[pos] = key;
+      perm[pos] = q;
+    }
   }
 }
 
@@ -1003,8 +1251,47 @@
   return EPA_OK;
 }
 
+int launch_build_lookup2f(epa_ctx* ctx) {
+  if (ctx->lookup2f || ctx->lookup2f_refused) return EPA_OK;
+  if (!ctx->lookup2) return epa_fail(ctx, EPA_ERR_INVALID_ARG, "the fp32 pair table needs the resident site-pair table");
+  const uint32_t BP = (ctx->B + 1) / 2, n = 2 * ((ctx->W + 1) / 2) * PE;
+  const size_t bytes = sizeof(float2) * (size_t)BP * n;
+  char* buf = nullptr;
+  constexpr size_t SCREEN_RESERVE = (size_t)4 << 30;
+  size_t free_b = 0, total_b = 0;
+  const bool room = hipMemGetInfo(&free_b, &total_b) == hipSuccess && free_b >= bytes + 16 + SCREEN_RESERVE;
+  if (!room || hipMalloc(&buf, bytes + 16) != hipSuccess) {
+    (void)hipGetLastError();
+    ctx->lookup2f_refused = true;
+    return EPA_OK;
+  }
+  uint32_t* stats = reinterpret_cast<uint32_t*>(buf + bytes);
+  EPA_HIP(ctx, hipMemsetAsync(stats, 0, 16, ctx->stream));
+  for (uint32_t p0 = 0; p0 < BP; p0 += EPA_GRID_Y)
+    hipLaunchKernelGGL(k_build_lookup2f, dim3((n + 255) / 256, std::min<uint32_t>(EPA_GRID_Y, BP - p0)), dim3(256), 0, ctx->stream,
+                       ctx->lookup2, ctx->W, ctx->B, reinterpret_cast<float2*>(buf), p0, stats);
+  uint32_t h[4] = {0, 0, 0, 0};
+  hipError_t e = hipGetLastError();
+  if (e == hipSuccess) e = hipMemcpyAsync(h, stats, 16, hipMemcpyDeviceToHost, ctx->stream);
+  if (e == hipSuccess) e = hipStreamSynchronize(ctx->stream);
+  if (e != hipSuccess) { (void)hipFree(buf); EPA_HIP(ctx, e); }
+  float m;
+  memcpy(&m, &h[0], 4);
+  ctx->screen_M = (double)m;
+  ctx->screen_nonfinite = h[1];
+  ctx->lookup2f = reinterpret_cast<float2*>(buf);
+  return EPA_OK;
+}
+
+double epa_screen_delta(const epa_ctx* ctx, uint32_t span_bound) {
+  if (!ctx->lookup2f || ctx->screen_nonfinite) return -1.0;
+  const double u = 0x1p-24, n = 2.0 * (span_bound >> 2) + 3.0;
+  const double delta = 2.0 * (n + 1.0) * u * n * ctx->screen_M * (double)std::max(ctx->opt.preplace_screen_scale, 1);
+  return delta <= 1.0 ? delta : -1.0;
+}
+
 int launch_preplace(epa_ctx* ctx, const uint8_t* d_codes, const uint32_t* d_begin, const uint32_t* d_span, uint32_t Q,
-                    const PreTable& t, uint32_t max_span, const uint32_t** d_status) {
+                    const PreTable& t, uint32_t max_span, const uint32_t** d_status, PreScreenProbe* probe) {
   double* const d_lnl = t.lnl;
   const uint32_t pitch = t.pitch, segp = t.segp;
   unsigned long long* const segmax = t.segmax;
@@ -1026,12 +1313,36 @@
   (void)rocprim::radix_sort_pairs<epa_radix_cfg>(nullptr, temp_bytes, (uint32_t*)nullptr, (uint32_t*)nullptr,
                                   (uint32_t*)nullptr, (uint32_t*)nullptr, Q, 0, 32, ctx->stream);
   uint32_t *status, *key_cnt, *iota, *sorted_keys, *perm, *keys;
+  const uint32_t nseg = (ctx->B + 63) / 64, seg32p = (nseg + 7u) & ~7u;
+  const uint32_t KB = 2 * Wp, n_blocks_c = 2 * nseg;
+  const uint64_t max_cells = (uint64_t)Q * nseg;
+  const uint32_t Kc = nseg * KB + 1;
+  const uint32_t max_runs_c = (uint32_t)std::min<uint64_t>((max_cells + GQ2 - 1) / GQ2 + n_blocks_c, 0xffffffu);
+  const uint32_t max_groups_c = max_runs_c + n_blocks_c * n_buckets;
+  const size_t smem_c = sizeof(uint32_t) * (2 * (n_blocks_c + 1) + 4 * (size_t)max_runs_c + 2);
+  double delta = -1.0;
+  constexpr uint64_t SCREEN_MIN_CELLS = 80000000ull;
+  const bool big = ctx->opt.preplace_screen >= 2 || probe || (uint64_t)Q * ctx->B >= SCREEN_MIN_CELLS;
+  if (pairs && !blocked && nseg <= 64 && max_span != 0 && max_span <= (uint32_t)CH && ctx->opt.preplace_screen && big &&
+      (probe || (segmax && t.band_t > 0.0)) && max_cells < 0x80000000ull && smem_c <= 65536) {
+    const int brc = launch_build_lookup2f(ctx);
+    if (brc) return brc;
+    delta = epa_screen_delta(ctx, span_bound);
+  }
+  const bool screen = delta >= 0.0;
+  uint32_t *seg32, *cstatus, *ccnt, *crank, *csorted, *cperm;
+  unsigned long long *seg_mask, *n_incl;
+  Group* cgroups;
   Group* groups;
   uint16_t *packed, *tails;
   void* temp;
   auto layout = [&](Carver c) {
     status = c.take<uint32_t>(64);
     key_cnt = c.take<uint32_t>(K);
+    seg32 = c.take<uint32_t>(screen ? (size_t)Q * seg32p : 0);
+    n_incl = c.take<unsigned long long>(screen ? 1 : 0);
+    cstatus = c.take<uint32_t>(screen ? 64 : 0);
+    ccnt = c.take<uint32_t>(screen ? Kc : 0);
     iota = c.take<uint32_t>(Q);
     sorted_keys = c.take<uint32_t>(Q);
     perm = c.take<uint32_t>(Q);
@@ -1039,6 +1350,11 @@
     groups = c.take<Group>(max_groups);
     packed = c.take<uint16_t>((size_t)Q * NP16);
     tails = c.take<uint16_t>((pairs || sites) ? 4 * (size_t)Q : 0);
+    seg_mask = c.take<unsigned long long>(screen ? Q : 0);
+    crank = c.take<uint32_t>(screen ? (size_t)Q * seg32p : 0);
+    csorted = c.take<uint32_t>(screen ? max_cells : 0);
+    cperm = c.take<uint32_t>(screen ? max_cells : 0);
+    cgroups = c.take<Group>(screen ? max_groups_c : 0);
     temp = c.tail(temp_bytes);
     return c.off;
   };
@@ -1097,8 +1413,8 @@
   const GenericKernel k_generic = sites ? nullptr : ctx->ncols == 16 ? (acc ? k_preplace<16, true> : k_preplace<16, false>) : (acc ? k_preplace<24, true> : k_preplace<24, false>);
   if (k_fast) EPA_HIP(ctx, hipFuncSetAttribute((const void*)k_fast, hipFuncAttributeMaxDynamicSharedMemorySize, (int)lds_fast));
   if (k_generic) EPA_HIP(ctx, hipFuncSetAttribute((const void*)k_generic, hipFuncAttributeMaxDynamicSharedMemorySize, (int)lds));
-  auto kernels = [&](const double* lk, const double* lk2, uint32_t nB, double* lnl, unsigned long long* sm) {
-    if (k_fast) {
+  auto kernels = [&](const double* lk, const double* lk2, uint32_t nB, double* lnl, unsigned long long* sm, bool fast = true) {
+    if (k_fast && fast) {
       const uint32_t tile = fast_acc ? (pairs ? NB2_ACC : NB2_ACC_S) : 16;
       const dim3 grid_f((uint32_t)std::min<uint64_t>((uint64_t)max_groups * ((nB + tile - 1) / tile), (uint64_t)ctx->n_cu));
       hipLaunchKernelGGL(k_fast, grid_f, dim3(GQ2), (uint32_t)lds_fast, ctx->stream, pairs ? lk2 : lk, (const uint16_t*)packed,
@@ -1112,6 +1428,58 @@
     hipLaunchKernelGGL(k_generic, grid, dim3(GQ), (uint32_t)lds, ctx->stream, lk, d_codes, d_begin, d_span, perm, groups, ctx->W,
                        cstride, crel, nB, pitch, codes_bytes, want_cls, status, lnl);
   };
+  if (probe) probe->ran = screen;
+  if (probe && !screen) return EPA_OK;
+  if (screen) {
+    using ScreenKernel = decltype(&k_preplace_screen<SPREAD, ROWL_NARROW>);
+    const ScreenKernel k_screen = wide ? k_preplace_screen<SPREAD_WIDE, ROWL_PACKED> : k_preplace_screen<SPREAD, ROWL_NARROW>;
+    const FastKernel k_exact = wide ? k_preplace_pairs<false, SPREAD_WIDE, ROWL_PACKED, true> : k_preplace_pairs<false, SPREAD, ROWL_NARROW, true>;
+    const size_t lds_scr = wide ? (size_t)((CH + SPREAD_WIDE) / 2) * ROWL_PACKED : (size_t)TROWS2 * ROWL_NARROW;
+    EPA_HIP(ctx, hipFuncSetAttribute((const void*)k_screen, hipFuncAttributeMaxDynamicSharedMemorySize, (int)lds_scr));
+    EPA_HIP(ctx, hipFuncSetAttribute((const void*)k_exact, hipFuncAttributeMaxDynamicSharedMemorySize, (int)lds_fast));
+    const uint32_t BP = (ctx->B + 1) / 2;
+    struct Events {
+      hipEvent_t e[3] = {nullptr, nullptr, nullptr};
+      ~Events() { for (hipEvent_t x : e) if (x) (void)hipEventDestroy(x); }
+    } evs;
+    hipEvent_t* const ev = evs.e;
+    if (probe) for (hipEvent_t& e : evs.e) EPA_HIP(ctx, hipEventCreate(&e));
+    if (probe) EPA_HIP(ctx, hipEventRecord(ev[0], ctx->stream));
+    else epa_timer_start(ctx, epa_t(ctx, epa_ctx::T_PREPLACE));
+    const dim3 grid_s((uint32_t)std::min<uint64_t>((uint64_t)max_groups * ((BP + 15) / 16), (uint64_t)ctx->n_cu));
+    hipLaunchKernelGGL(k_screen, grid_s, dim3(GQ2), (uint32_t)lds_scr, ctx->stream, (const float2*)ctx->lookup2f, (const uint16_t*)packed,
+                       (const uint16_t*)tails, d_begin, d_span, perm, groups, ctx->W, BP, NP16, status, seg32, seg32p);
+    if (probe) EPA_HIP(ctx, hipEventRecord(ev[1], ctx->stream));
+    const double band = (probe ? probe->band_t : t.band_t) + 2.0 * delta;
+    hipLaunchKernelGGL(k_screen_band, dim3((Q + 255) / 256), dim3(256), 0, ctx->stream, (const uint32_t*)seg32, Q, nseg, seg32p, band,
+                       delta, (const uint32_t*)keys, KB, probe ? nullptr : segmax, segp, probe ? nullptr : ccnt, crank, seg_mask, n_incl);
+    if (probe) {
+      EPA_HIP(ctx, hipEventRecord(ev[2], ctx->stream));
+      EPA_HIP(ctx, hipGetLastError());
+      EPA_HIP(ctx, hipEventSynchronize(ev[2]));
+      (void)hipEventElapsedTime(&probe->ms_screen, ev[0], ev[1]);
+      (void)hipEventElapsedTime(&probe->ms_band, ev[1], ev[2]);
+      probe->delta = delta;
+      probe->seg32 = seg32;
+      probe->mask = seg_mask;
+      probe->n_incl = n_incl;
+      return EPA_OK;
+    }
+    ++ctx->screen_runs;
+    launch_scan_counts(ctx, ccnt, Kc);
+    hipLaunchKernelGGL(k_scatter_cells, dim3((Q + 255) / 256), dim3(256), 0, ctx->stream, (const unsigned long long*)seg_mask,
+                       (const uint32_t*)keys, (const uint32_t*)crank, (const uint32_t*)ccnt, Q, seg32p, KB, (uint32_t)max_cells, csorted, cperm);
+    hipLaunchKernelGGL(k_make_groups, dim3(1), dim3(256), smem_c, ctx->stream, (const uint32_t*)csorted, (uint32_t)max_cells, Wp, n_blocks_c,
+                       n_blocks_c, (uint32_t)GQ2, (uint32_t)GQ2, (uint32_t)(wide ? SPREAD_WIDE : SPREAD), max_runs_c, cgroups, max_groups_c,
+                       cstatus, (const uint32_t*)(ccnt + (Kc - 1)), KB);
+    hipLaunchKernelGGL(k_exact, dim3(std::min<uint32_t>(max_groups_c, (uint32_t)ctx->n_cu)), dim3(GQ2), (uint32_t)lds_fast, ctx->stream,
+                       (const double*)ctx->lookup2, (const uint16_t*)packed, (const uint16_t*)tails, d_begin, d_span, (const uint32_t*)cperm,
+                       (const Group*)cgroups, ctx->W, ctx->B, pitch, NP16, (const uint32_t*)cstatus, d_lnl, segmax, segp);
+    kernels(ctx->lookup, ctx->lookup2, ctx->B, d_lnl, segmax, false);
+    epa_timer_stop(ctx, epa_t(ctx, epa_ctx::T_PREPLACE));
+    EPA_HIP(ctx, hipGetLastError());
+    return EPA_OK;
+  }
   if (!blocked) {
     epa_timer_start(ctx, epa_t(ctx, epa_ctx::T_PREPLACE));
     kernels(ctx->lookup, ctx->lookup2, ctx->B, d_lnl, segmax);
diff --git a/epa_ng_amd/csrc/select.hip b/epa_ng_amd/csrc/select.hip
--- a/epa_ng_amd/csrc/select.hip
+++ b/epa_ng_amd/csrc/select.hip
@@ -623,6 +623,15 @@
 
 }
 
+static bool select_bitmap_form(const epa_ctx* ctx, uint32_t Q) {
+  return !ctx->opt.select_sort && (size_t)ctx->B * ((Q + 31) / 32) * sizeof(uint32_t) <= ((size_t)64 << 20);
+}
+
+bool epa_select_takes_seg(const epa_ctx* ctx, const PreTable& t, uint32_t Q, double threshold) {
+  return select_bitmap_form(ctx, Q) && t.segmax && !ctx->opt.select_full_rows && ctx->heur_mode == 0 && threshold < 1.0 &&
+         (ctx->B + 63) / 64 <= 64;
+}
+
 int launch_select_begin(epa_ctx* ctx, const PreTable& t, const uint32_t* pre_status, uint32_t Q, double threshold,
                         epa_pair* d_pairs, uint64_t max_pairs, const uint32_t* d_span, uint32_t* rb, SelectPending* sp) {
   sp->have_hist = false;
@@ -645,7 +654,7 @@
   (void)rocprim::radix_sort_keys<epa_radix_cfg>(nullptr, sort_bytes, (unsigned long long*)nullptr,
                                  (unsigned long long*)nullptr, worst, 0, 64, ctx->stream);
   const uint32_t wpr = (Q + 31) / 32;
-  const bool bm = !ctx->opt.select_sort && (size_t)B * wpr * sizeof(uint32_t) <= ((size_t)64 << 20);
+  const bool bm = select_bitmap_form(ctx, Q);
   uint32_t* status = nullptr;
   size_t fill = 0;
   auto layout = [&](Carver c) {
@@ -684,9 +693,8 @@
   epa_timer_start(ctx, epa_t(ctx, epa_ctx::T_SELECT));
   auto select_rows = [&](const SelOut& so) -> bool {
     const int nr = (int)((B + 63) / 64);
-    if (so.bitmap && t.segmax && !ctx->opt.select_full_rows && mode == 0 && threshold < 1.0 && nr <= 64) {
-      const double band_x = 1.0 - std::log((1.0 - threshold) / (double)B);
-      const double band_t = std::max(band_x, std::log((double)B) + 38.0);
+    if (so.bitmap && epa_select_takes_seg(ctx, t, Q, threshold)) {
+      const double band_x = epa_select_band_x(threshold, B), band_t = epa_select_band_t(threshold, B);
       constexpr uint32_t sel_grid = 16;
       const dim3 grid_seg(std::min<uint32_t>((Q + 3) / 4, (uint32_t)ctx->n_cu * sel_grid));
       hipLaunchKernelGGL(k_select_seg<8>, grid_seg, dim3(256), 0, ctx->stream, d_lnl, t.segmax, t.segp, Q, B, pitch, threshold,
diff --git a/include/epa_dev.h b/include/epa_dev.h
--- a/include/epa_dev.h
+++ b/include/epa_dev.h
@@ -161,6 +161,11 @@
 
 int epa_dev_preplace_bounded(epa_ctx* ctx, const uint8_t* q_codes, const uint32_t* win_begin,
                              const uint32_t* win_span, uint32_t Q, uint32_t max_span, double* lnl, uint64_t* seg_keys);
+
+int epa_dev_preplace_screen_probe(epa_ctx* ctx, const uint8_t* q_codes, const uint32_t* win_begin,
+                                  const uint32_t* win_span, uint32_t Q, uint32_t max_span, double threshold,
+                                  float* seg32, uint64_t* seg_mask, double* info);
+uint64_t epa_dev_preplace_screen_runs(const epa_ctx* ctx);
 
 int epa_dev_thorough(epa_ctx* ctx, const epa_pair* pairs, uint64_t n_pairs,
                      const uint8_t* q_codes, const uint32_t* win_begin, const uint32_t* win_span,
```

Result: faster. 17.97 million placements/s, median of 6 (+2.1%).
